# eloimoliner/audio-inpainting-diffusion

Hardware: AMD Instinct MI355X
Metric: denoiser-steps/sec (higher is better)
Workload: dtype f32; 1 GPU; BASELINE.json configs[1]: batch 8 x 22.05 kHz MAESTRO-shape segments (L=184184) per GPU, 300 ms gap, T=36 EDM schedule, Heun steps 5..16; branch=xi=0.25 (reconstruction guidance: forward + input-VJP), segments_per_gpu=8, network=unet_cqt_oct_with_attention 7-octave, 186.3 M params, random-init (seeded), sub_batch_streams=2, cu_partition=0, hip_graph_replay=False, backend=single process, visible_gpus=1

## Files before the change

audio_inpainting_diffusion_amd/_lib.py:

```python
from __future__ import annotations

import ctypes as C
import os
from typing import Optional, Sequence

import torch

_HERE = os.path.dirname(os.path.abspath(__file__))
LIB_PATH = os.path.join(_HERE, "libaid_hip.so")
if os.environ.get("AID_EXPERIMENT") == "1" and os.environ.get("AID_LIB_PATH"):
    LIB_PATH = os.environ["AID_LIB_PATH"]
    import sys as _sys
    print(f"[aid] AID_EXPERIMENT=1: loading {LIB_PATH} instead of the in-tree libaid_hip.so", file=_sys.stderr)
AID_CQT_MAX_OCT = 12
AID_STATS_SPLIT = 32
AID_CONV2D_SPLIT_FLAG_BYTES = 4096
AID_ATTN_MAX_T = 128


class AidError(RuntimeError):
    pass


class View(C.Structure):
# ... 21 lines not shown
                ("dot_ws", C.c_void_p), ("dot_n", C.c_int), ("stat_ws", C.c_void_p), ("stat_n", C.c_int),
                ("x2", View), ("Cin1", C.c_int),
                ("fin_mode", C.c_int), ("fin_count", C.c_void_p), ("fin_gamma", C.c_void_p), ("fin_mod", C.c_void_p), ("fin_mod_ld", C.c_int64),
                ("fin_eps", C.c_float), ("fin_scale", C.c_void_p), ("fin_stats", C.c_void_p)]


class Wino2dGemmParams(C.Structure):
    _fields_ = [("U", C.c_void_p), ("V", C.c_void_p), ("M", C.c_void_p), ("nxi", C.c_int), ("Cin", C.c_int), ("Cout", C.c_int),
                ("Cin_pad", C.c_int), ("Cout_pad", C.c_int), ("N", C.c_int64), ("variant", C.c_int)]


class ResampleParams(C.Structure):
    _fields_ = [("x", View), ("y", View), ("B", C.c_int), ("C", C.c_int), ("F", C.c_int), ("T", C.c_int),
                ("up", C.c_int), ("adjoint", C.c_int), ("accumulate", C.c_int)]


class AttentionParams(C.Structure):
    _fields_ = [("qk", C.c_void_p), ("v", C.c_void_p), ("out", C.c_void_p), ("probs", C.c_void_p),
                ("B", C.c_int), ("H", C.c_int), ("F", C.c_int), ("T", C.c_int), ("scale", C.c_float), ("bias", C.c_void_p)]


class EmbedParams(C.Structure):
    _fields_ = [("sigma", C.c_void_p), ("rff_freq", C.c_void_p), ("w0", C.c_void_p), ("b0", C.c_void_p),
                ("w1", C.c_void_p), ("b1", C.c_void_p), ("w2", C.c_void_p), ("b2", C.c_void_p), ("emb", C.c_void_p),
                ("B", C.c_int), ("rff", C.c_int), ("h0", C.c_int), ("h1", C.c_int), ("E", C.c_int)]


class ModulationParams(C.Structure):
    _fields_ = [("emb", C.c_void_p), ("W", C.c_void_p), ("bias", C.c_void_p), ("mod", C.c_void_p),
                ("B", C.c_int), ("E", C.c_int), ("N", C.c_int)]


class CqtTables(C.Structure):
    _fields_ = [("n_oct", C.c_int), ("bins", C.c_int), ("rc", C.c_void_p), ("Lg", C.c_void_p), ("goff", C.c_void_p),
                ("g", C.c_void_p), ("T_oct", C.c_void_p), ("twiddle", C.c_void_p), ("Tmax", C.c_int)]


class CqtParams(C.Structure):
    _fields_ = [("tab", CqtTables), ("T_host", C.c_int * AID_CQT_MAX_OCT), ("oct", View * AID_CQT_MAX_OCT),
                ("spec", C.c_void_p), ("band_ws", C.c_void_p), ("in_scale", C.c_void_p), ("B", C.c_int), ("Lh", C.c_int),
                ("unnormalized", C.c_int)]


class CqtGatherParams(C.Structure):
    _fields_ = [("band_ws", C.c_void_p), ("kfirst", C.c_void_p), ("kcount", C.c_void_p),
                ("rc", C.c_void_p), ("Lg", C.c_void_p), ("goff", C.c_void_p), ("woff", C.c_void_p), ("Tk", C.c_void_p),
                ("gdM", C.c_void_p), ("X", C.c_void_p), ("cskip", C.c_void_p), ("cout", C.c_void_p), ("hpf", C.c_void_p),
                ("Y", C.c_void_p), ("B", C.c_int), ("Lh", C.c_int), ("ws_per_b", C.c_int64), ("band_scale", C.c_void_p)]


class AxpbyParams(C.Structure):
    _fields_ = [("x", C.c_void_p), ("y", C.c_void_p), ("out", C.c_void_p), ("a", C.c_void_p), ("b", C.c_void_p),
                ("B", C.c_int), ("L", C.c_int64), ("a_host", C.c_float), ("b_host", C.c_float)]

    def __init__(self, x, y, out, a, b, B, L, a_host=1.0, b_host=1.0):
        super().__init__(x, y, out, a, b, B, L, a_host, b_host)


class ScoreStepParams(C.Structure):
    _fields_ = [("x", C.c_void_p), ("xhat", C.c_void_p), ("yobs", C.c_void_p), ("smask", C.c_void_p),
                ("smask_sB", C.c_int64), ("x0", C.c_void_p), ("d0", C.c_void_p), ("t", C.c_void_p), ("h", C.c_void_p),
                ("xnext", C.c_void_p), ("dout", C.c_void_p), ("xh_out", C.c_void_p),
                ("B", C.c_int), ("L", C.c_int64), ("mode", C.c_int), ("t_host", C.c_float), ("h_host", C.c_float)]


class Add2Params(C.Structure):
    _fields_ = [("u", View), ("v", View), ("y", View), ("B", C.c_int), ("C", C.c_int), ("F", C.c_int), ("T", C.c_int),
                ("a", C.c_float), ("b", C.c_float)]


class ScaleActParams(C.Structure):
    _fields_ = [("x", View), ("y", View), ("scale", C.c_void_p), ("scale_ld", C.c_int64),
                ("B", C.c_int), ("C", C.c_int), ("F", C.c_int), ("T", C.c_int), ("act", C.c_int), ("wino", C.c_int), ("dilF", C.c_int), ("mul", C.c_float)]


class FftPassParams(C.Structure):
    _fields_ = [("inp", C.c_void_p), ("out", C.c_void_p), ("twiddle", C.c_void_p), ("B", C.c_int), ("N", C.c_int), ("R", C.c_int),
                ("Ns", C.c_int), ("in_mode", C.c_int), ("out_mode", C.c_int), ("sign", C.c_float), ("out_scale", C.c_float)]


class GroupDotParams(C.Structure):
    _fields_ = [("u", View), ("v", View), ("B", C.c_int), ("C", C.c_int), ("F", C.c_int), ("T", C.c_int), ("groups", C.c_int),
                ("ws", C.c_void_p)]


class NormBwdParams(C.Structure):
    _fields_ = [("gd", View), ("x", View), ("gy", View), ("out", View),
                ("B", C.c_int), ("C", C.c_int), ("F", C.c_int), ("T", C.c_int), ("groups", C.c_int),
                ("stats", C.c_void_p), ("ws", C.c_void_p), ("eps", C.c_float), ("a", C.c_float), ("accumulate", C.c_int),
                ("ws_n", C.c_int), ("wout", View), ("wscale", C.c_void_p), ("wscale_ld", C.c_int64), ("wform", C.c_int), ("coef_ready", C.c_int), ("wdil", C.c_int)]


class AttentionBwdParams(C.Structure):
    _fields_ = [("qk", C.c_void_p), ("v", C.c_void_p), ("probs", C.c_void_p), ("gout", C.c_void_p),
                ("gqk", C.c_void_p), ("gv", C.c_void_p), ("B", C.c_int), ("H", C.c_int), ("F", C.c_int), ("T", C.c_int),
                ("scale", C.c_float), ("accumulate_gv", C.c_int), ("ws", C.c_void_p)]


class GuidanceSeedParams(C.Structure):
    _fields_ = [("xhat", C.c_void_p), ("y", C.c_void_p), ("mask", C.c_void_p), ("mask_sB", C.c_int64),
                ("g", C.c_void_p), ("norm", C.c_void_p), ("B", C.c_int), ("L", C.c_int64), ("norm_type", C.c_int), ("beta", C.c_float)]

    def __init__(self, xhat, y, mask, mask_sB, g, norm, B, L, norm_type=2, beta=1.0):
        super().__init__(xhat, y, mask, mask_sB, g, norm, B, L, norm_type, beta)


class GuidanceStepParams(C.Structure):
    _fields_ = [("xhat", C.c_void_p), ("g", C.c_void_p), ("out", C.c_void_p), ("step_out", C.c_void_p), ("s_out", C.c_void_p),
                ("B", C.c_int), ("L", C.c_int64), ("coef", C.c_float), ("inv_sqrt_len", C.c_float), ("eps", C.c_float)]


class SetRowsParams(C.Structure):
    _fields_ = [("out", C.c_void_p), ("ld", C.c_int64), ("B", C.c_int), ("n", C.c_int), ("v", C.c_float * 8)]


class RowNormParams(C.Structure):
    _fields_ = [("x", C.c_void_p), ("out", C.c_void_p), ("B", C.c_int), ("L", C.c_int64)]


class ResamplePolyParams(C.Structure):
    _fields_ = [("x", C.c_void_p), ("y", C.c_void_p), ("kernel", C.c_void_p), ("x_ld", C.c_int64), ("y_ld", C.c_int64),
                ("L", C.c_int64), ("Lout", C.c_int64), ("B", C.c_int), ("orig_freq", C.c_int), ("new_freq", C.c_int),
                ("width", C.c_int), ("K", C.c_int)]


class StftParams(C.Structure):
    _fields_ = [("x", C.c_void_p), ("frames", C.c_void_p), ("out", C.c_void_p),
                ("window", C.c_void_p), ("twiddle", C.c_void_p), ("inv_env", C.c_void_p),
                ("mask", C.c_void_p), ("mask_sB", C.c_int64), ("mask_ld", C.c_int64),
                ("add1", C.c_void_p), ("add2", C.c_void_p), ("c0", C.c_float),
                ("B", C.c_int), ("L", C.c_int64), ("Lp", C.c_int64),
                ("n_fft", C.c_int), ("hop", C.c_int), ("n_frames", C.c_int), ("adjoint", C.c_int)]


class WgradParams(C.Structure):
    _fields_ = [("gy", View), ("x", View), ("P", C.c_void_p),
                ("B", C.c_int), ("Cin", C.c_int), ("Cout", C.c_int), ("F", C.c_int), ("T", C.c_int), ("KH", C.c_int), ("KW", C.c_int),
                ("dilF", C.c_int), ("S", C.c_int), ("alpha", C.c_float), ("wino", C.c_int)]


class WinoGyParams(C.Structure):
    _fields_ = [("gy", View), ("out", View), ("B", C.c_int), ("C", C.c_int), ("F", C.c_int), ("T", C.c_int)]


class PackConvWeightParams(C.Structure):
    _fields_ = [("w", C.c_void_p), ("wp", C.c_void_p), ("wpT", C.c_void_p), ("wpw", C.c_void_p), ("wpwT", C.c_void_p),
                ("Cout", C.c_int), ("Cin", C.c_int), ("KH", C.c_int), ("KW", C.c_int),
                ("Cin_pad", C.c_int), ("Cout_pad", C.c_int), ("Cin_padT", C.c_int), ("Cout_padT", C.c_int),
                ("wpw8", C.c_void_p), ("wpw8T", C.c_void_p), ("wpw2", C.c_void_p), ("wpw2T", C.c_void_p), ("wpw3", C.c_void_p), ("wpw3T", C.c_void_p)]


class WgradReduceParams(C.Structure):
    _fields_ = [("P", C.c_void_p), ("W", C.c_void_p), ("gate", C.c_void_p), ("gate_ld", C.c_int64),
                ("in_scale", C.c_void_p), ("in_scale_ld", C.c_int64), ("dW", C.c_void_p), ("dgate", C.c_void_p), ("dgate_ld", C.c_int64),
                ("B", C.c_int), ("S", C.c_int), ("Cout", C.c_int), ("Cin", C.c_int), ("K", C.c_int), ("accumulate", C.c_int),
                ("wino", C.c_int), ("Uw", C.c_void_p), ("Cin_pad", C.c_int), ("Cout_pad", C.c_int)]


class ChannelDotParams(C.Structure):
    _fields_ = [("u", View), ("v", View), ("out", C.c_void_p), ("out_ld", C.c_int64),
                ("B", C.c_int), ("C", C.c_int), ("F", C.c_int), ("T", C.c_int)]


class RelposBwdParams(C.Structure):
    _fields_ = [("dS", C.c_void_p), ("bucket", C.c_void_p), ("dW", C.c_void_p),
                ("B", C.c_int), ("H", C.c_int), ("T", C.c_int), ("num_buckets", C.c_int), ("accumulate", C.c_int)]


class ScaleBwdParams(C.Structure):
    _fields_ = [("S", C.c_void_p), ("S_ld", C.c_int64), ("scale", C.c_void_p), ("scale_ld", C.c_int64), ("gamma", C.c_void_p),
                ("mod", C.c_void_p), ("mod_ld", C.c_int64), ("stats", C.c_void_p), ("dgamma", C.c_void_p), ("dmod", C.c_void_p),
                ("dmod_ld", C.c_int64), ("B", C.c_int), ("C", C.c_int), ("groups", C.c_int), ("accumulate", C.c_int)]


class ModulationBwdParams(C.Structure):
    _fields_ = [("dmod", C.c_void_p), ("emb", C.c_void_p), ("W", C.c_void_p), ("dW", C.c_void_p), ("dbias", C.c_void_p),
                ("demb", C.c_void_p), ("B", C.c_int), ("E", C.c_int), ("N", C.c_int), ("accumulate", C.c_int),
                ("part", C.c_void_p), ("part_floats", C.c_int64)]


class EmbedBwdParams(C.Structure):
    _fields_ = [("fwd", EmbedParams), ("demb", C.c_void_p), ("dw0", C.c_void_p), ("db0", C.c_void_p), ("dw1", C.c_void_p),
                ("db1", C.c_void_p), ("dw2", C.c_void_p), ("db2", C.c_void_p), ("accumulate", C.c_int)]


class AdamParams(C.Structure):
    _fields_ = [("param", C.c_void_p), ("grad", C.c_void_p), ("m", C.c_void_p), ("v", C.c_void_p), ("gscale", C.c_void_p),
                ("n", C.c_int64), ("lr", C.c_float), ("beta1", C.c_float), ("beta2", C.c_float), ("eps", C.c_float),
                ("bias1", C.c_float), ("bias2_sqrt", C.c_float)]


class EmaParams(C.Structure):
    _fields_ = [("dst", C.c_void_p), ("src", C.c_void_p), ("n", C.c_int64), ("rate", C.c_float)]


class SumsqParams(C.Structure):
    _fields_ = [("x", C.c_void_p), ("ws", C.c_void_p), ("out", C.c_void_p), ("n", C.c_int64), ("max_norm", C.c_float)]


AID_SUMSQ_BLOCKS = 512


class FirParams(C.Structure):
    _fields_ = [("x", C.c_void_p), ("out", C.c_void_p), ("h", C.c_void_p), ("add1", C.c_void_p), ("add2", C.c_void_p), ("c0", C.c_float),
                ("B", C.c_int), ("K", C.c_int), ("stride", C.c_int), ("pad_left", C.c_int), ("adjoint", C.c_int),
                ("L", C.c_int64), ("L_out", C.c_int64), ("x_ld", C.c_int64), ("out_ld", C.c_int64)]


class IirParams(C.Structure):
    _fields_ = [("x", C.c_void_p), ("out", C.c_void_p), ("pre", C.c_void_p), ("coef", C.c_void_p), ("H", C.c_void_p),
                ("z", C.c_void_p), ("state", C.c_void_p), ("add1", C.c_void_p), ("add2", C.c_void_p), ("c0", C.c_float),
                ("B", C.c_int), ("N", C.c_int), ("C", C.c_int), ("clamp", C.c_int), ("adjoint", C.c_int),
                ("L", C.c_int64), ("x_ld", C.c_int64), ("out_ld", C.c_int64)]


class ClipParams(C.Structure):
    _fields_ = [("x", C.c_void_p), ("xref", C.c_void_p), ("out", C.c_void_p), ("add1", C.c_void_p), ("add2", C.c_void_p),
                ("c0", C.c_float), ("clip", C.c_float), ("B", C.c_int), ("adjoint", C.c_int),
                ("L", C.c_int64), ("x_ld", C.c_int64), ("out_ld", C.c_int64)]


AID_DEGRADE_ABI_VERSION = 1
DEGRADE_EXPORTS = ["aid_degrade_abi_version", "aid_fir", "aid_iir", "aid_clip"]


class StftMagParams(C.Structure):
    _fields_ = [("x", C.c_void_p), ("g", C.c_void_p), ("out", C.c_void_p), ("frames", C.c_void_p), ("window", C.c_void_p), ("twiddle", C.c_void_p),
                ("B", C.c_int), ("n_fft", C.c_int), ("hop", C.c_int), ("n_frames", C.c_int), ("adjoint", C.c_int),
                ("L", C.c_int64), ("x_ld", C.c_int64), ("out_ld", C.c_int64)]


class MatrixNormParams(C.Structure):
    _fields_ = [("den", C.c_void_p), ("y", C.c_void_p), ("g", C.c_void_p), ("norm", C.c_void_p), ("r", C.c_void_p), ("diag", C.c_void_p),
                ("B", C.c_int), ("F", C.c_int), ("T", C.c_int), ("ord", C.c_int), ("max_iter", C.c_int), ("tol", C.c_double)]


AID_PHASE_ABI_VERSION = 1
PHASE_EXPORTS = ["aid_phase_abi_version", "aid_stft_mag", "aid_matrix_norm_seed"]

class ArCarryParams(C.Structure):
    _fields_ = [("x", C.c_void_p), ("y", C.c_void_p), ("out", C.c_void_p), ("B", C.c_int), ("first", C.c_int),
                ("L", C.c_int64), ("end", C.c_int64), ("off", C.c_int64), ("out_ld", C.c_int64)]


AID_AR_ABI_VERSION = 1
AR_EXPORTS = ["aid_ar_abi_version", "aid_ar_carry"]


class WindowGatherParams(C.Structure):
    _fields_ = [("rec", C.c_void_p), ("out", C.c_void_p), ("mask", C.c_void_p), ("y", C.c_void_p), ("m", C.c_void_p), ("jobs", C.c_void_p),
                ("J", C.c_int), ("R", C.c_int), ("L", C.c_int64), ("N", C.c_int64), ("rec_ld", C.c_int64), ("out_ld", C.c_int64), ("mask_ld", C.c_int64)]


class WindowScatterParams(C.Structure):
    _fields_ = [("x", C.c_void_p), ("out", C.c_void_p), ("jobs", C.c_void_p), ("J", C.c_int), ("R", C.c_int),
                ("L", C.c_int64), ("N", C.c_int64), ("out_ld", C.c_int64)]


AID_RESTORE_ABI_VERSION = 1
AID_RESTORE_JOB_FIELDS = 6
RESTORE_EXPORTS = ["aid_restore_abi_version", "aid_window_gather", "aid_window_scatter"]

class ClipKnownParams(C.Structure):
    _fields_ = [("x", C.c_void_p), ("xref", C.c_void_p), ("y", C.c_void_p), ("state", C.c_void_p), ("clip", C.c_void_p), ("out", C.c_void_p),
                ("B", C.c_int), ("mode", C.c_int), ("L", C.c_int64), ("x_ld", C.c_int64), ("xref_ld", C.c_int64), ("y_ld", C.c_int64),
                ("state_ld", C.c_int64), ("out_ld", C.c_int64)]


class DeclipGatherParams(C.Structure):
    _fields_ = [("rec", C.c_void_p), ("out", C.c_void_p), ("clip", C.c_void_p), ("y", C.c_void_p), ("k", C.c_void_p), ("c", C.c_void_p), ("jobs", C.c_void_p),
                ("J", C.c_int), ("R", C.c_int), ("L", C.c_int64), ("N", C.c_int64), ("rec_ld", C.c_int64), ("out_ld", C.c_int64)]


AID_DECLIP_ABI_VERSION = 1
DECLIP_EXPORTS = ["aid_declip_abi_version", "aid_clip_known", "aid_declip_gather"]

class ResamplePolyAdjParams(C.Structure):
    _fields_ = [("g", C.c_void_p), ("gx", C.c_void_p), ("kT", C.c_void_p), ("j_lo", C.c_void_p), ("j_hi", C.c_void_p),
                ("g_ld", C.c_int64), ("gx_ld", C.c_int64), ("L", C.c_int64), ("Lout", C.c_int64),
                ("B", C.c_int), ("orig_freq", C.c_int), ("new_freq", C.c_int), ("width", C.c_int), ("K", C.c_int)]


AID_RESAMPLE_OP_ABI_VERSION = 1
RESAMPLE_OP_EXPORTS = ["aid_resample_op_abi_version", "aid_resample_poly_adj"]

class FirObservedParams(C.Structure):
    _fields_ = [("x", C.c_void_p), ("y", C.c_void_p), ("state", C.c_void_p), ("h", C.c_void_p), ("out", C.c_void_p),
                ("B", C.c_int), ("K", C.c_int), ("mode", C.c_int), ("L", C.c_int64), ("x_ld", C.c_int64), ("y_ld", C.c_int64),
                ("state_ld", C.c_int64), ("out_ld", C.c_int64)]


class BweGatherParams(C.Structure):
    _fields_ = [("rec", C.c_void_p), ("out", C.c_void_p), ("y", C.c_void_p), ("state", C.c_void_p), ("jobs", C.c_void_p),
                ("J", C.c_int), ("R", C.c_int), ("K", C.c_int), ("L", C.c_int64), ("N", C.c_int64), ("rec_ld", C.c_int64), ("out_ld", C.c_int64)]


AID_BWE_LONG_ABI_VERSION = 1
BWE_LONG_EXPORTS = ["aid_bwe_long_abi_version", "aid_fir_observed", "aid_bwe_gather"]

EXPORTS = ["aid_abi_version", "aid_last_error", "aid_last_kernel", "aid_group_stats", "aid_conv2d", "aid_conv2d_pack_dims", "aid_conv2d_stat_partials", "aid_pack_conv_weight", "aid_wino_gy", "aid_conv2d_wgrad_tiles", "aid_resample",
           "aid_time_attention", "aid_embed", "aid_modulation", "aid_cqt_analysis", "aid_cqt_synthesis",
           "aid_cqt_gather", "aid_axpby", "aid_score_step", "aid_add2", "aid_group_dot", "aid_norm_bwd",
           "aid_time_attention_bwd", "aid_guidance_seed", "aid_guidance_step", "aid_set_rows", "aid_row_norm", "aid_scale_act", "aid_fft_pass",
           "aid_stft_frames", "aid_stft_ola", "aid_resample_poly", "aid_conv2d_wino_input_supported", "aid_conv2d_dot_partials", "aid_conv2d_x2_supported", "aid_conv2d_dot_partials_1x1", "aid_conv2d_wino_input_ok", "aid_conv2d_wino_form", "aid_conv2d_wino8_supported", "aid_conv2d_wino_split_ws_bytes", "aid_conv2d_fin_supported",
           "aid_conv2d_wgrad", "aid_wgrad_reduce", "aid_channel_dot", "aid_relpos_bwd", "aid_scale_bwd", "aid_modulation_bwd", "aid_embed_bwd",
           "aid_adam", "aid_ema", "aid_sumsq", "aid_wino2d_gemm", "aid_wino2d_set_split", "aid_conv2d_wino2d_gemm", "aid_conv2d_wino2d_output", "aid_conv2d_wino2d_supported", "aid_conv2d_wino2d_positions", "aid_conv2d_wino2d_wanted", "aid_conv2d_wino2d_tform"]

_lib = None


def lib():
    global _lib
    if _lib is None:
        if not os.path.exists(LIB_PATH):
            raise AidError(f"{LIB_PATH} not found: build the HIP extension first (python __graft_entry__.py). "
                           "There is no CPU / eager fallback on the product path.")
        L = C.CDLL(LIB_PATH)
        L.aid_last_error.restype = C.c_char_p
        L.aid_abi_version.restype = C.c_int
        L.aid_last_kernel.restype = C.c_char_p
        for name in EXPORTS:
            if not hasattr(L, name):
                raise AidError(f"libaid_hip.so does not export {name}")
        L.aid_conv2d_pack_dims.argtypes = [C.c_int, C.c_int, C.POINTER(C.c_int), C.POINTER(C.c_int)]
        L.aid_conv2d_pack_dims.restype = None
        L.aid_conv2d_wino_input_supported.argtypes = [C.c_int, C.c_int, C.c_int]
        L.aid_conv2d_wino_input_supported.restype = C.c_int
        L.aid_conv2d_dot_partials.argtypes = [C.c_int] * 7
        L.aid_conv2d_dot_partials.restype = C.c_int
        L.aid_conv2d_x2_supported.argtypes = [C.c_int] * 5
        L.aid_conv2d_x2_supported.restype = C.c_int
        L.aid_conv2d_dot_partials_1x1.argtypes = [C.c_int] * 5
        L.aid_conv2d_dot_partials_1x1.restype = C.c_int
        L.aid_conv2d_wino_input_ok.argtypes = [C.c_int] * 6
        L.aid_conv2d_wino_input_ok.restype = C.c_int
        L.aid_conv2d_wino8_supported.argtypes = [C.c_int] * 5
        L.aid_conv2d_wino8_supported.restype = C.c_int
        L.aid_conv2d_fin_supported.argtypes = [C.c_int] * 7
        L.aid_conv2d_fin_supported.restype = C.c_int
        L.aid_conv2d_wino_form.argtypes = [C.c_int] * 6
        L.aid_conv2d_wino_form.restype = C.c_int
        L.aid_conv2d_wino_split_ws_bytes.argtypes = [C.c_int] * 6
        L.aid_conv2d_wino_split_ws_bytes.restype = C.c_int64
        L.aid_conv2d_stat_partials.argtypes = [C.c_int] * 7
        L.aid_conv2d_stat_partials.restype = C.c_int
        L.aid_conv2d_wgrad_tiles.argtypes = [C.c_int] * 5
        L.aid_conv2d_wgrad_tiles.restype = C.c_int
        L.aid_conv2d_wino2d_supported.argtypes = [C.c_int] * 5
        L.aid_conv2d_wino2d_supported.restype = C.c_int
        L.aid_conv2d_wino2d_wanted.argtypes = [C.c_int] * 6
        L.aid_conv2d_wino2d_wanted.restype = C.c_int
        L.aid_conv2d_wino2d_tform.argtypes = [C.c_int] * 6
        L.aid_conv2d_wino2d_tform.restype = C.c_int
        L.aid_conv2d_wino2d_positions.argtypes = [C.c_int] * 4
        L.aid_conv2d_wino2d_positions.restype = C.c_int64
        L.aid_wino2d_set_split.argtypes = [C.c_int]
        L.aid_wino2d_set_split.restype = C.c_int
        for name in EXPORTS[3:]:
            if name not in ("aid_conv2d_pack_dims", "aid_conv2d_wino_input_supported", "aid_conv2d_dot_partials", "aid_conv2d_x2_supported", "aid_conv2d_dot_partials_1x1", "aid_conv2d_wino_input_ok", "aid_conv2d_wino_form", "aid_conv2d_wino8_supported", "aid_conv2d_wino_split_ws_bytes", "aid_conv2d_fin_supported",
                            "aid_conv2d_stat_partials", "aid_conv2d_wgrad_tiles", "aid_conv2d_wino2d_supported", "aid_conv2d_wino2d_positions", "aid_conv2d_wino2d_wanted", "aid_conv2d_wino2d_tform", "aid_wino2d_set_split"):
                getattr(L, name).argtypes = [C.c_void_p, C.c_void_p]
                getattr(L, name).restype = C.c_int
        if L.aid_abi_version() != 14:
            raise AidError("ABI version mismatch")
        for name in DEGRADE_EXPORTS:
            if not hasattr(L, name):
                raise AidError(f"libaid_hip.so does not export {name}")
            getattr(L, name).argtypes = [C.c_void_p, C.c_void_p]
            getattr(L, name).restype = C.c_int
        L.aid_degrade_abi_version.argtypes = []
        if L.aid_degrade_abi_version() != AID_DEGRADE_ABI_VERSION:
            raise AidError("include/aid_degrade.h ABI version mismatch")
        for name in PHASE_EXPORTS:
            if not hasattr(L, name):
                raise AidError(f"libaid_hip.so does not export {name}")
            getattr(L, name).argtypes = [C.c_void_p, C.c_void_p]
            getattr(L, name).restype = C.c_int
        L.aid_phase_abi_version.argtypes = []
        if L.aid_phase_abi_version() != AID_PHASE_ABI_VERSION:
            raise AidError("include/aid_phase.h ABI version mismatch")
        for name in AR_EXPORTS:
            if not hasattr(L, name):
                raise AidError(f"libaid_hip.so does not export {name}")
            getattr(L, name).argtypes = [C.c_void_p, C.c_void_p]
            getattr(L, name).restype = C.c_int
        L.aid_ar_abi_version.argtypes = []
        if L.aid_ar_abi_version() != AID_AR_ABI_VERSION:
            raise AidError("include/aid_autoregressive.h ABI version mismatch")
        for name in RESTORE_EXPORTS:
            if not hasattr(L, name):
                raise AidError(f"libaid_hip.so does not export {name}")
            getattr(L, name).argtypes = [C.c_void_p, C.c_void_p]
            getattr(L, name).restype = C.c_int
        L.aid_restore_abi_version.argtypes = []
        if L.aid_restore_abi_version() != AID_RESTORE_ABI_VERSION:
            raise AidError("include/aid_restore.h ABI version mismatch")
        for name in DECLIP_EXPORTS:
            if not hasattr(L, name):
                raise AidError(f"libaid_hip.so does not export {name}")
            getattr(L, name).argtypes = [C.c_void_p, C.c_void_p]
            getattr(L, name).restype = C.c_int
        L.aid_declip_abi_version.argtypes = []
        if L.aid_declip_abi_version() != AID_DECLIP_ABI_VERSION:
            raise AidError("include/aid_declip.h ABI version mismatch")
        for name in RESAMPLE_OP_EXPORTS:
            if not hasattr(L, name):
                raise AidError(f"libaid_hip.so does not export {name}")
            getattr(L, name).argtypes = [C.c_void_p, C.c_void_p]
            getattr(L, name).restype = C.c_int
        L.aid_resample_op_abi_version.argtypes = []
        if L.aid_resample_op_abi_version() != AID_RESAMPLE_OP_ABI_VERSION:
            raise AidError("include/aid_resample_op.h ABI version mismatch")
        for name in BWE_LONG_EXPORTS:
            if not hasattr(L, name):
                raise AidError(f"libaid_hip.so does not export {name}")
            getattr(L, name).argtypes = [C.c_void_p, C.c_void_p]
            getattr(L, name).restype = C.c_int
        L.aid_bwe_long_abi_version.argtypes = []
        if L.aid_bwe_long_abi_version() != AID_BWE_LONG_ABI_VERSION:
            raise AidError("include/aid_bwe_long.h ABI version mismatch")
        _lib = L
    return _lib


def _stream() -> int:
    return torch.cuda.current_stream().cuda_stream


def call(name: str, params) -> None:
    rc = getattr(lib(), name)(C.addressof(params), _stream())
    if rc != 0:
        raise AidError(f"{name} failed rc={rc}: {lib().aid_last_error().decode()}")


def call_on(fn, params_addr: int, stream: int, name: str = "") -> None:
    rc = fn(params_addr, stream)
    if rc != 0:
        raise AidError(f"{name} failed rc={rc}: {lib().aid_last_error().decode()}")


def _req(t: torch.Tensor):
    if not (t.is_cuda and t.dtype == torch.float32):
        raise AidError("HIP kernels need float32 tensors on the GPU (no CPU fallback)")


def ptr(t: Optional[torch.Tensor]) -> Optional[int]:
    return None if t is None else t.data_ptr()


def view4(t: Optional[torch.Tensor]) -> View:
    if t is None:
        return View(None, 0, 0, 0)
    _req(t)
    assert t.dim() == 4 and (t.stride(3) == 1 or t.shape[3] == 1), "T must be contiguous"
    return View(t.data_ptr(), t.stride(0), t.stride(1), t.stride(2))


def pack_dims(cin: int, cout: int):
    a, b = C.c_int(0), C.c_int(0)
    lib().aid_conv2d_pack_dims(cin, cout, C.byref(a), C.byref(b))
    return a.value, b.value


def pack_conv_weight(w: torch.Tensor, transpose: bool = False) -> torch.Tensor:
    if w.dim() == 2:
        w = w[:, :, None, None]
    elif w.dim() == 3:
        w = w[:, :, None, :]
    w = w.detach().float()
    if transpose:
        w = w.flip(2, 3).permute(1, 0, 2, 3)
    co, ci, kh, kw = w.shape
    cip, cop = pack_dims(ci, co)
    out = torch.zeros(kh * kw, cip, cop, device=w.device, dtype=torch.float32)
    out[:, :ci, :co] = w.permute(2, 3, 1, 0).reshape(kh * kw, ci, co)
    return out


def pack_conv_weight_wino(w: torch.Tensor, transpose: bool = False) -> torch.Tensor:
    w = w.detach().double()
    if transpose:
        w = w.flip(2, 3).permute(1, 0, 2, 3)
    co, ci, kh, kw = w.shape
    assert (kh, kw) == (5, 3)
    w0, w1, w2 = w[..., 0], w[..., 1], w[..., 2]
    U = torch.stack((w0 / 4, -(w0 + w1 + w2) / 6, -(w0 - w1 + w2) / 6, (w0 + 2 * w1 + 4 * w2) / 24,
                     (w0 - 2 * w1 + 4 * w2) / 24, w2), dim=0)
    nxi = U.shape[0]
    cip, cop = pack_dims(ci, co)
    out = torch.zeros(nxi * kh, cip, cop, device=w.device, dtype=torch.float32)
    out[:, :ci, :co] = U.permute(0, 3, 2, 1).reshape(nxi * kh, ci, co).float()
    return out


W8_POINTS = (0.4, 0.8, 1.25, 2.5)


def wino8_matrices():
    import numpy as np
    n = 10
    pts = np.array([0.0] + [sg * a for a in W8_POINTS for sg in (1, -1)], dtype=np.float64)

    def vander(cols):
        V = np.zeros((n, cols))
        for j in range(n - 1):
            V[j] = pts[j] ** np.arange(cols)
        V[n - 1, cols - 1] = 1.0
        return V
    AT, G, BT = vander(8).T, vander(3), np.linalg.inv(vander(n)).T
    sc = np.abs(BT).max(axis=1)
    BT = BT / sc[:, None]
    BT[np.abs(BT) < 1e-13] = 0.0
    return AT, G * sc[:, None], BT


def wino45_matrices():
    import numpy as np

    def toom(points, m, r):
        n = m + r - 1
        pts = np.array([0.0] + [sg * a for a in points for sg in (1, -1)], dtype=np.float64)

        def vander(cols):
            V = np.zeros((n, cols))
            for j in range(n - 1):
                V[j] = pts[j] ** np.arange(cols)
            V[n - 1, cols - 1] = 1.0
            return V
        AT, G, BT = vander(m).T, vander(r), np.linalg.inv(vander(n)).T
        sc = np.abs(BT).max(axis=1)
        BT = BT / sc[:, None]
        BT[np.abs(BT) < 1e-13] = 0.0
        return AT, G * sc[:, None], BT
    return toom((1.0, 2.0, 0.5), 4, 5) + toom((1.0, 2.0), 4, 3)


def pack_conv_weight_wino2d(w: torch.Tensor, transpose: bool = False) -> torch.Tensor:
    w = w.detach().double()
    if transpose:
        w = w.flip(2, 3).permute(1, 0, 2, 3)
    co, ci, kh, kw = w.shape
    assert (kh, kw) == (5, 3)
    m = wino45_matrices()
    GF, GT = torch.from_numpy(m[1]).to(w.device), torch.from_numpy(m[4]).to(w.device)
    U = torch.einsum("fh,tk,oihk->ftio", GF, GT, w).reshape(48, ci, co)
    cip, cop = pack_dims(ci, co)
    out = torch.zeros(48, cip, cop, device=w.device, dtype=torch.float32)
    out[:, :ci, :co] = U.float()
    return out


def pack_conv_weight_wino2d8(w: torch.Tensor, transpose: bool = False) -> torch.Tensor:
    w = w.detach().double()
    if transpose:
        w = w.flip(2, 3).permute(1, 0, 2, 3)
    co, ci, kh, kw = w.shape
    assert (kh, kw) == (5, 3)
    GF = torch.from_numpy(wino45_matrices()[1]).to(w.device)
    G8 = torch.from_numpy(wino8_matrices()[1]).to(w.device)
    U = torch.einsum("fh,tk,oihk->ftio", GF, G8, w).reshape(80, ci, co)
    cip, cop = pack_dims(ci, co)
    out = torch.zeros(80, cip, cop, device=w.device, dtype=torch.float32)
    out[:, :ci, :co] = U.float()
    return out


def pack_conv_weight_wino8(w: torch.Tensor, transpose: bool = False) -> torch.Tensor:
    w = w.detach().double()
    if transpose:
        w = w.flip(2, 3).permute(1, 0, 2, 3)
    co, ci, kh, kw = w.shape
    assert (kh, kw) == (5, 3)
    G = torch.from_numpy(wino8_matrices()[1]).to(w.device)
    U = torch.einsum("xk,oihk->xoih", G, w)
    cip, cop = pack_dims(ci, co)
    out = torch.zeros(10 * kh, cip, cop, device=w.device, dtype=torch.float32)
    out[:, :ci, :co] = U.permute(0, 3, 2, 1).reshape(10 * kh, ci, co).float()
    return out


def _cqt_params(tr, tab, octs: Sequence[torch.Tensor], window: Optional[torch.Tensor] = None) -> CqtParams:
    P = tr.plan
    p = CqtParams()
    p.tab = CqtTables(P.numocts, P.binsoct, ptr(tab["rc"]), ptr(tab["Lg"]), ptr(tab["goff"]),
                      ptr(tab["g"] if window is None else window), ptr(tab["T_oct"]), ptr(tab["twiddle"]), P.Tmax)
    for o in range(P.numocts):
        p.T_host[o] = int(P.T_oct[o])
        t = octs[o]
        _req(t)
        assert t.shape[1] == 2 and t.shape[2] == P.binsoct and t.shape[3] == P.T_oct[o] and t.stride(3) == 1
        p.oct[o] = View(t.data_ptr(), t.stride(0), t.stride(1), t.stride(2))
    p.B = octs[0].shape[0]
    p.Lh = P.Lh
    p.unnormalized = 0
    return p


def cqt_analysis(tr, tab, spec_ri: torch.Tensor, octs, in_scale=None, window=None, unnormalized=False):
    _req(spec_ri)
    assert spec_ri.is_contiguous()
    p = _cqt_params(tr, tab, octs, window)
    p.spec = spec_ri.data_ptr()
    p.in_scale = ptr(in_scale)
    p.unnormalized = int(unnormalized)
    call("aid_cqt_analysis", p)


def cqt_synthesis(tr, tab, octs, ws: torch.Tensor):
    p = _cqt_params(tr, tab, octs)
    p.band_ws = ws.data_ptr()
    call("aid_cqt_synthesis", p)


def cqt_gather(tr, tab, ws, Y, X=None, cskip=None, cout=None, hpf=None, window=None, band_scale=None):
    P = tr.plan
    p = CqtGatherParams(ptr(ws), ptr(tab["kfirst"]), ptr(tab["kcount"]), ptr(tab["rc"]), ptr(tab["Lg"]),
                        ptr(tab["goff"]), ptr(tab["woff"]), ptr(tab["Tk"]), ptr(tab["gdM"] if window is None else window),
                        ptr(X), ptr(cskip), ptr(cout), ptr(hpf), Y.data_ptr(), Y.shape[0], P.Lh, P.ws_per_b, ptr(band_scale))
    call("aid_cqt_gather", p)
```

audio_inpainting_diffusion_amd/csrc/aid_conv.hip:

```cpp
#include "aid_common.h"
#include "aid_mfma_dma.h"
#include "aid_conv1x1_plan.h"
#include <stdlib.h>

struct ConvDev {
    aid_conv2d_params p;
    int tt_log2;
    int rows_log2;
    int tiles_t;
    int nrows;
    int nchunks;
    int splits, cps;
    float* ws;
};

__device__ __forceinline__ float4 xform4(float4 v, float sc, int act) {
    v.x *= sc; v.y *= sc; v.z *= sc; v.w *= sc;
    if (act == 1) { v.x = aid_gelu(v.x); v.y = aid_gelu(v.y); v.z = aid_gelu(v.z); v.w = aid_gelu(v.w); }
    return v;
}

template <int KH, int KW, int MT, int NT, int WGM, int WGN, int KC>
__global__ __launch_bounds__(64 * WGM * WGN) void conv_mfma_kernel(const ConvDev a) {
    constexpr int NTHREADS = 64 * WGM * WGN;
// ... 137 lines not shown
            const bool ok = xg[i] >= 0 && c < p.Cin;
            xv[i] = ok ? *reinterpret_cast<const float4*>(p.x.p + xg[i] + (int64_t)c * p.x.sC) : make_float4(0.f, 0.f, 0.f, 0.f);
            xs[i] = (ok && p.in_scale) ? p.in_scale[xsc[i] + c] : 1.f;
        }
        if (KW > 1) {
#pragma unroll
            for (int i = 0; i < HQ; ++i) {
                const int c = c0 + hci[i];
                const bool ok = hg[i] >= 0 && c < p.Cin;
                float v = ok ? p.x.p[hg[i] + (int64_t)c * p.x.sC] : 0.f;
                if (ok && p.in_scale) v *= p.in_scale[hsc[i] + c];
                hv[i] = v;
            }
        }
#pragma unroll
        for (int i = 0; i < WQ; ++i)
            wv[i] = (wg[i] >= 0) ? *reinterpret_cast<const float4*>(wbase + wg[i] + (int64_t)c0 * p.Cout_pad)
                                 : make_float4(0.f, 0.f, 0.f, 0.f);
    };
    auto write_slot = [&](float* Xs, float* Ws, int slot) {
#pragma unroll
        for (int i = 0; i < XQ; ++i)
            if ((slot < 0 || (i % (NSLOT - 1)) == slot) && (XQ_TOTAL % NTHREADS == 0 || xlds[i] >= 0))
                *reinterpret_cast<float4*>(Xs + xlds[i]) = xform4(xv[i], xs[i], p.act);
#pragma unroll
        for (int i = 0; i < WQ; ++i)
            if ((slot < 0 || (i % (NSLOT - 1)) == slot) && wlds[i] >= 0)
                *reinterpret_cast<float4*>(Ws + wlds[i]) = wv[i];
        if (KW > 1 && (slot < 0 || slot == NSLOT - 2)) {
#pragma unroll
            for (int i = 0; i < HQ; ++i)
                if (hlds[i] >= 0) Xs[hlds[i]] = (p.act == 1) ? aid_gelu(hv[i]) : hv[i];
        }
    };
    auto halo_slow = [&](float* Xs, int c0) {
        for (int h = tid; h < 2 * nstrips; h += NTHREADS) {
            const int s = h >> 1, side = h & 1;
            const int kh = s % KH;
            const int s2 = s / KH;
            const int rr = s2 & (ROWS - 1);
            const int ci = s2 >> a.rows_log2;
            const int b = rowinfo[2 * rr];
            const int fi = rowinfo[2 * rr + 1] + (kh - KH / 2) * p.dilF;
            const int t = side ? (t0 + TT) : (t0 - 1);
            const int c = c0 + ci;
            float v = 0.f;
            if (b >= 0 && fi >= 0 && fi < p.F && c < p.Cin && t >= 0 && t < p.T) {
                v = p.x.p[(int64_t)b * p.x.sB + (int64_t)c * p.x.sC + (int64_t)fi * p.x.sF + t];
                if (p.in_scale) v *= p.in_scale[(int64_t)b * p.in_scale_ld + c];
                if (p.act == 1) v = aid_gelu(v);
            }
            Xs[s * TTP + (side ? 4 + TT : 3)] = v;
        }
    };

    const int cb = (int)blockIdx.z * a.cps;
    const int nloc = (a.nchunks - cb < a.cps) ? (a.nchunks - cb) : a.cps;
    issue_loads(cb * KC);
    write_slot(smem, smem + XSZ, -1);
    if (KW > 1 && !halo_fast) halo_slow(smem, cb * KC);
    __syncthreads();

    for (int ch = 0; ch < nloc; ++ch) {
        const int cur = ch & 1;
        const float* Xs = smem + cur * BUFSZ;
        const float* Ws = Xs + XSZ;
        float* Xn = smem + (cur ^ 1) * BUFSZ;
        float* Wn = Xn + XSZ;
        const bool more = (ch + 1) < nloc;
        float av[2][MT], bv[2][NT];
        auto load_frags = [&](int ks, int buf) {
            const int tap = ks / (KC / 2);
            const int cp = ks % (KC / 2);
            const int kh = tap / KW, kw = tap % KW;
            const int ci = 2 * cp + ci_lane;
#pragma unroll
            for (int i = 0; i < MT; ++i)
                av[buf][i] = Ws[(tap * KC + ci) * M_BLK + (wm * MT + i) * 32 + (lane & 31)];
#pragma unroll
            for (int j = 0; j < NT; ++j)
                bv[buf][j] = Xs[ci * strip_ci + kh * TTP + xoff[j] + kw];
        };
        load_frags(0, 0);
#pragma unroll
        for (int slot = 0; slot < NSLOT; ++slot) {
            if (slot == 0) __builtin_amdgcn_s_setprio(3);
            else if (slot == 1) __builtin_amdgcn_s_setprio(2);
            else if (slot == 2) __builtin_amdgcn_s_setprio(1);
            else __builtin_amdgcn_s_setprio(0);
#pragma unroll
            for (int k = 0; k < KS_PER_SLOT; ++k) {
                const int ks = slot * KS_PER_SLOT + k;
                if (ks + 1 < KSTEPS) load_frags(ks + 1, (ks + 1) & 1);
#pragma unroll
                for (int i = 0; i < MT; ++i)
#pragma unroll
                    for (int j = 0; j < NT; ++j)
                        acc[i][j] = __builtin_amdgcn_mfma_f32_32x32x2f32(av[ks & 1][i], bv[ks & 1][j], acc[i][j], 0, 0, 0);
                if (slot == 0 && k == 0 && more) issue_loads((cb + ch + 1) * KC);
            }
            if (more && slot > 0) write_slot(Xn, Wn, slot - 1);
        }
        if (more && KW > 1 && !halo_fast) halo_slow(Xn, (cb + ch + 1) * KC);
        __syncthreads();
    }

#pragma unroll
    for (int j = 0; j < NT; ++j) {
        const int n = (wn * NT + j) * 32 + (lane & 31);
        const int rr = n >> a.tt_log2;
        const int tt = n & (TT - 1);
        const int b = rowinfo[2 * rr];
        const int f = rowinfo[2 * rr + 1];
        const int t = t0 + tt;
        if (b < 0 || t >= p.T) continue;
        if (a.splits > 1) {
            const int64_t ft = (int64_t)p.F * p.T;
            float* wsb = a.ws + (((int64_t)blockIdx.z * p.B + b) * p.Cout) * ft + (int64_t)f * p.T + t;
#pragma unroll
            for (int i = 0; i < MT; ++i) {
                const int mbase = m0 + (wm * MT + i) * 32 + 4 * (lane >> 5);
#pragma unroll
                for (int r = 0; r < 16; ++r) {
                    const int m = mbase + (r & 3) + 8 * (r >> 2);
                    if (m < p.Cout) wsb[(int64_t)m * ft] = acc[i][j][r];
                }
            }
            continue;
        }
        const int64_t ybase = (int64_t)b * p.y.sB + (int64_t)f * p.y.sF + t;
        const int64_t rbase = p.res.p ? ((int64_t)b * p.res.sB + (int64_t)f * p.res.sF + t) : 0;
        const int64_t abase = p.aux.p ? ((int64_t)b * p.aux.sB + (int64_t)f * p.aux.sF + t) : 0;
#pragma unroll
        for (int i = 0; i < MT; ++i) {
            float rv[16], uv[16], sv[16];
            const int mbase = m0 + (wm * MT + i) * 32 + 4 * (lane >> 5);
#pragma unroll
            for (int r = 0; r < 16; ++r) {
                const int m = mbase + (r & 3) + 8 * (r >> 2);
                const bool ok = m < p.Cout;
                rv[r] = (ok && p.res.p) ? p.res.p[rbase + (int64_t)m * p.res.sC] : 0.f;
                sv[r] = (ok && p.out_scale) ? p.out_scale[(int64_t)b * p.out_scale_ld + m] : 1.f;
                uv[r] = (ok && p.epi == 1) ? p.aux.p[abase + (int64_t)m * p.aux.sC] * p.aux_scale[(int64_t)b * p.aux_scale_ld + m] : 0.f;
            }
#pragma unroll
            for (int r = 0; r < 16; ++r) {
                const int m = mbase + (r & 3) + 8 * (r >> 2);
                if (m >= p.Cout) continue;
                float v = acc[i][j][r] * sv[r];
                if (p.epi == 1) v *= aid_dgelu(uv[r]);
                v += p.res_scale * rv[r];
                p.y.p[ybase + (int64_t)m * p.y.sC] = p.alpha * v;
            }
        }
    }
}

__global__ __launch_bounds__(256) void conv_splitk_reduce_kernel(const aid_conv2d_params p, const float* __restrict__ ws, int splits) {
    const int64_t ft = (int64_t)p.F * p.T;
    const int64_t q4 = ft >> 2;
    const int64_t total = (int64_t)p.B * p.Cout * q4;
    const int64_t i = (int64_t)blockIdx.x * 256 + threadIdx.x;
    if (i >= total) return;
    const int64_t bm = i / q4, e = (i - bm * q4) * 4;
    const int b = (int)(bm / p.Cout), m = (int)(bm - (int64_t)b * p.Cout);
    const int f = (int)(e / p.T), t = (int)(e - (int64_t)f * p.T);
    const int64_t plane = (int64_t)p.B * p.Cout * ft;
    float4 s = make_float4(0.f, 0.f, 0.f, 0.f);
    for (int z = 0; z < splits; ++z) {
        const float4 v = *reinterpret_cast<const float4*>(ws + z * plane + bm * ft + e);
        s.x += v.x; s.y += v.y; s.z += v.z; s.w += v.w;
    }
    const float sc = p.out_scale ? p.out_scale[(int64_t)b * p.out_scale_ld + m] : 1.f;
    float4 r = make_float4(0.f, 0.f, 0.f, 0.f);
    if (p.res.p) r = *reinterpret_cast<const float4*>(p.res.p + (int64_t)b * p.res.sB + (int64_t)m * p.res.sC + (int64_t)f * p.res.sF + t);
    float4 o;
    o.x = p.alpha * (p.res_scale * r.x + s.x * sc); o.y = p.alpha * (p.res_scale * r.y + s.y * sc);
    o.z = p.alpha * (p.res_scale * r.z + s.z * sc); o.w = p.alpha * (p.res_scale * r.w + s.w * sc);
    *reinterpret_cast<float4*>(p.y.p + (int64_t)b * p.y.sB + (int64_t)m * p.y.sC + (int64_t)f * p.y.sF + t) = o;
}

int aid_conv_splitk_reduce(const aid_conv2d_params* p, const float* ws, int splits, hipStream_t st) {
    const int64_t total = (int64_t)p->B * p->Cout * ((int64_t)p->F * p->T / 4);
    hipLaunchKernelGGL(conv_splitk_reduce_kernel, dim3((unsigned)((total + 255) / 256)), dim3(256), 0, st, *p, ws, splits);
    AID_CHECK_LAUNCH();
    return AID_OK;
}

bool aid_conv_splitk_scratch_ok(const aid_conv2d_params* p, int S) {
    return p->ws && c11_splitk_fits(S, p->B, p->Cout, p->F, p->T, p->ws_bytes) && aid_view_aligned(p->y, 4) && (!p->res.p || aid_view_aligned(p->res, 4));
}

extern "C" void aid_conv2d_pack_dims(int Cin, int Cout, int* Cin_pad, int* Cout_pad) {
    const int mb = c11_pick_mblk(Cout);
    *Cin_pad = ((Cin + 31) / 32) * 32;
    *Cout_pad = ((Cout + mb - 1) / mb) * mb;
}

template <int KH, int KW, int MT, int NT, int WGM, int WGN, int KC>
static int launch_cfg(const aid_conv2d_params* p, hipStream_t st, int splits = 1) {
    constexpr int M_BLK = 32 * MT * WGM;
    constexpr int N_BLK = 32 * NT * WGN;
    ConvDev a;
    a.p = *p;
    int TT = aid_pow2ceil(p->T);
    if (TT > N_BLK) TT = N_BLK;
    if (TT < 4) TT = 4;
    a.tt_log2 = aid_ilog2(TT);
    const int ROWS = N_BLK / TT;
    a.rows_log2 = aid_ilog2(ROWS);
    a.tiles_t = aid_cdiv(p->T, TT);
    a.nrows = p->B * p->F;
    a.nchunks = aid_cdiv(p->Cin, KC);
    a.cps = aid_cdiv(a.nchunks, splits);
    a.splits = aid_cdiv(a.nchunks, a.cps);
    a.ws = p->ws;
    const int rgroups = aid_cdiv(a.nrows, ROWS);
    dim3 grid((unsigned)(rgroups * a.tiles_t), (unsigned)(p->Cout_pad / M_BLK), (unsigned)a.splits);
    const size_t lds = sizeof(float) * 2 * ((size_t)KC * ROWS * KH * (TT + (KW > 1 ? 8 : 0)) + (size_t)KH * KW * KC * M_BLK) +
                       sizeof(int) * 2 * ROWS;
    AID_REQUIRE(lds <= 160 * 1024, "aid_conv2d: LDS tile too large");
    auto kern = conv_mfma_kernel<KH, KW, MT, NT, WGM, WGN, KC>;
    static bool attr_set = false;
    if (!attr_set) {
        (void)hipFuncSetAttribute((const void*)kern, hipFuncAttributeMaxDynamicSharedMemorySize, 160 * 1024);
        attr_set = true;
    }
    hipLaunchKernelGGL(kern, grid, dim3(64 * WGM * WGN), lds, st, a);
    AID_CHECK_LAUNCH();
    aid_note_kernel(a.splits > 1 ? "conv_mfma_kernel+splitk" : (KH == 5 ? "conv_mfma_kernel(5x3)" : "conv_mfma_kernel(1x1)"));
    if (a.splits > 1) return aid_conv_splitk_reduce(p, (const float*)p->ws, a.splits, st);
    return AID_OK;
}

static int launch_m53(const aid_conv2d_params* p, hipStream_t st) {
    int mb = c11_pick_mblk(p->Cout);
    if (mb == 128) {
        const int64_t npos = (int64_t)p->B * p->F * p->T;
        const int64_t ntiles = (npos + 255) / 256;
        if (ntiles * (p->Cout_pad / 128) < 192) mb = (ntiles * (p->Cout_pad / 64) < 192) ? 32 : 64;
    }
    switch (mb) {
        case 32: return launch_cfg<5, 3, 1, 2, 1, 4, 4>(p, st);
        case 64:
            if (p->T >= 64) return launch_cfg<5, 3, 1, 2, 2, 8, 4>(p, st);
            return launch_cfg<5, 3, 2, 2, 1, 4, 4>(p, st);
        case 96: return launch_cfg<5, 3, 1, 2, 3, 4, 4>(p, st);
        default: return launch_cfg<5, 3, 1, 2, 4, 4, 4>(p, st);
    }
}

template <int KC>
static int launch_m11(const aid_conv2d_params* p, hipStream_t st) {
    C11Shape s = c11_shape_of(*p);
    C11Plan pl = c11_tiled_plan(s);
    if (pl.S > 1 && !aid_conv_splitk_scratch_ok(p, pl.S)) {
        s.ws = false;
        pl = c11_tiled_plan(s);
    }
    AID_REQUIRE(pl.ok, "aid_conv2d: too many rows or tiles for the tiled 1x1 kernel");
    if (pl.S > 1) return launch_cfg<1, 1, 1, 2, 2, 4, KC>(p, st, pl.S);
    switch (pl.WGM) {
        case 1: return launch_cfg<1, 1, 1, 2, 1, 4, KC>(p, st);
        case 2: return launch_cfg<1, 1, 1, 2, 2, 4, KC>(p, st);
        case 3: return launch_cfg<1, 1, 1, 2, 3, 4, KC>(p, st);
        default: return launch_cfg<1, 1, 1, 2, 4, 4, KC>(p, st);
    }
}

int aid_conv53_dma_try(const aid_conv2d_params* p, hipStream_t st);
int aid_conv53_wino_try(const aid_conv2d_params* p, hipStream_t st);
int aid_conv53_wino2d(const aid_conv2d_params* p, hipStream_t st);
int aid_conv1x1_stream_try(const aid_conv2d_params* p, hipStream_t st);
int aid_conv1x1_dma_try(const aid_conv2d_params* p, hipStream_t st);
int aid_conv_small_try(const aid_conv2d_params* p, hipStream_t st);
int aid_conv1x1_rs_try(const aid_conv2d_params* p, hipStream_t st);

static int conv1x1_dispatch(const aid_conv2d_params* p, hipStream_t st, const char* only_first_two) {
    int r = aid_conv1x1_rs_try(p, st);
    if (r == 0) r = aid_conv1x1_dma_try(p, st);
    if (r == 0 && only_first_two) {
        aid_set_error(only_first_two);
        return AID_E_BADARG;
    }
    if (r == 0) r = aid_conv1x1_stream_try(p, st);
    if (r != 0) return r < 0 ? r : AID_OK;
    return p->Cin <= 8 ? launch_m11<8>(p, st) : launch_m11<16>(p, st);
}

static C11Shape c11_query_shape(int B, int Cin, int Cout, int F, int T) {
    C11Shape s = {};
    int cip;
    aid_conv2d_pack_dims(Cin, Cout, &cip, &s.Cout_pad);
    s.B = B; s.Cin = Cin; s.Cout = Cout; s.F = F; s.T = T;
    return s;
}

extern "C" int aid_conv2d_dot_partials_1x1(int B, int Cin, int Cout, int F, int T) {
    C11Shape s = c11_query_shape(B, Cin, Cout, F, T);
    s.epi = 1; s.dot = true;
    return c11_plan(s).slots;
}

extern "C" int aid_conv2d_x2_supported(int Cin, int Cin1, int Cout, int F, int T) {
    C11Shape s = c11_query_shape(1, Cin, Cout, F, T);
    s.x2 = true; s.Cin1 = Cin1;
    return c11_dma_plan(s).family ? 1 : 0;
}

extern "C" int aid_conv2d(const aid_conv2d_params* p, void* stream) {
    hipStream_t st = (hipStream_t)stream;
    AID_REQUIRE(p && p->x.p && p->y.p && p->wp, "aid_conv2d: null pointer");
    AID_REQUIRE(p->B > 0 && p->Cin > 0 && p->Cout > 0 && p->F > 0 && p->T > 0, "aid_conv2d: empty shape");
    AID_REQUIRE((p->T % 4) == 0, "aid_conv2d: T must be a multiple of 4");
    AID_REQUIRE(p->x_wino == 3 || p->x_wino == 4 || aid_view_strides(p->x, 4), "aid_conv2d: input view strides % 4 == 0");
    AID_REQUIRE((((uintptr_t)p->x.p) & 15) == 0, "aid_conv2d: input view must be 16-byte aligned");
    int cip, cop;
    aid_conv2d_pack_dims(p->Cin, p->Cout, &cip, &cop);
    AID_REQUIRE(p->Cin_pad == cip && p->Cout_pad == cop, "aid_conv2d: packed weight dims mismatch (use aid_conv2d_pack_dims)");
    AID_REQUIRE(p->epi == 0 || (p->epi == 1 && p->aux.p && p->aux_scale), "aid_conv2d: epi=1 needs aux + aux_scale");
    AID_REQUIRE((int64_t)p->B * p->in_scale_ld < (1LL << 31), "aid_conv2d: in_scale too large");
    AID_REQUIRE(!p->x_wino || (p->KH == 5 && p->KW == 3 && p->wp_wino), "aid_conv2d: x_wino is a 5x3 Winograd-path input layout");
    AID_REQUIRE(!p->fin_mode || (p->x_wino && p->KH == 5 && p->KW == 3), "aid_conv2d: fin_mode is an option of the row-shared 5x3 Winograd kernels (aid_conv2d_fin_supported)");
    if (p->x_wino == 3 || p->x_wino == 4) return aid_conv53_wino2d(p, st);
    if (p->x2.p) {
        AID_REQUIRE(p->KH == 1 && p->KW == 1 && !p->in_scale && p->act == 0 && p->Cin1 > 0 && p->Cin1 < p->Cin && (p->Cin1 % 16) == 0 && ((p->Cin - p->Cin1) % 16) == 0,
                    "aid_conv2d: x2 is an option of plain 1x1 convolutions with both K segments multiples of 16");
        return conv1x1_dispatch(p, st, "aid_conv2d: x2 given but the layer is not eligible for the 1x1 kernels that take it");
    }
    if (p->stat_ws) {
        AID_REQUIRE(!p->dot_ws && p->epi == 0 && p->x_wino, "aid_conv2d: stat_ws is an option of the forward epilogue on Winograd-domain input");
        AID_REQUIRE(p->stat_n > 0 && p->stat_n == aid_conv2d_stat_partials(p->B, p->Cin, p->Cout, p->F, p->T, p->dilF, p->x_wino), "aid_conv2d: stat_n != aid_conv2d_stat_partials()");
    }
    if (p->dot_ws && p->KH == 1 && p->KW == 1) {
        AID_REQUIRE(p->epi == 1 && !p->res.p, "aid_conv2d: dot_ws on a 1x1 layer is an option of the dGELU epilogue without residual");
        return conv1x1_dispatch(p, st, "aid_conv2d: dot_ws given but the 1x1 layer is not eligible (aid_conv2d_dot_partials_1x1)");
    }
    if (p->dot_ws) {
        AID_REQUIRE(p->KH == 5 && p->KW == 3 && p->wp_wino && p->wino_taps == (p->x_wino == 2 ? 50 : 30) && p->epi == 1 && !p->res.p,
                    "aid_conv2d: dot_ws is an option of the F(4,3) / F(8,3) dGELU epilogue");
        AID_REQUIRE(p->dot_n > 0 && p->dot_n == aid_conv2d_dot_partials(p->B, p->Cin, p->Cout, p->F, p->T, p->dilF, p->x_wino), "aid_conv2d: dot_n != aid_conv2d_dot_partials()");
        const int r = aid_conv53_wino_try(p, st);
        if (r == 0) aid_set_error("aid_conv2d: dot_ws given but the layer is not eligible for the F(4,3) kernels");
        return r == 1 ? AID_OK : (r < 0 ? r : AID_E_BADARG);
    }
    if (p->x_wino) {
        const int r = aid_conv53_wino_try(p, st);
        return r == 1 ? AID_OK : (r < 0 ? r : AID_E_BADARG);
    }
    if (p->Cin <= 8 || p->Cout <= 8) {
        const int r = aid_conv_small_try(p, st);
        if (r != 0) return r < 0 ? r : AID_OK;
    }
    if (p->KH == 5 && p->KW == 3) {
        if (p->wp_wino) {
            const int r = aid_conv53_wino_try(p, st);
            if (r != 0) return r < 0 ? r : AID_OK;
        }
        {
            const int r = aid_conv53_dma_try(p, st);
            if (r != 0) return r < 0 ? r : AID_OK;
        }
        return launch_m53(p, st);
    }
    if (p->KH == 1 && p->KW == 1) return conv1x1_dispatch(p, st, nullptr);
    aid_set_error("aid_conv2d: unsupported kernel size (5x3 and 1x1 only)");
    return AID_E_BADARG;
}
```

audio_inpainting_diffusion_amd/csrc/aid_conv1x1_dma.hip:

```cpp
#include "aid_common.h"
#include "aid_mfma_dma.h"
#include "aid_conv1x1_plan.h"
#include <type_traits>

int aid_conv_splitk_reduce(const aid_conv2d_params* p, const float* ws, int splits, hipStream_t st);
bool aid_conv_splitk_scratch_ok(const aid_conv2d_params* p, int S);

struct C11Dev {
    aid_conv2d_params p;
    const float* zero;
    int tt_log2, rows_log2, tiles_t, nrows, nchunks;
    int nx, ny, per_xcd;
    int nch1;
    int splits, cps;
    float* ws;
};

__device__ float4 g_aid_zero_page_c11[16];

template <int MT, int WGM, int WGN, int RMAX, int KC, int MINW>
__global__ __launch_bounds__(64 * WGM * WGN, MINW) void conv11_dma_kernel(const C11Dev a) {
    constexpr int NT = 2;
    constexpr int NW = WGM * WGN;
    constexpr int NTHREADS = 64 * NW;
    constexpr int M_BLK = 32 * MT * WGM;
    constexpr int N_BLK = 32 * NT * WGN;
    constexpr int XSZ = KC * N_BLK;
    constexpr int WROW = (M_BLK % 64 == 0) ? M_BLK : ((M_BLK + 63) / 64) * 64;
    constexpr int WSZ = KC * WROW;
    constexpr int BUFSZ = XSZ + WSZ;
    constexpr int NXP = XSZ / 256;
    constexpr int NWP = WSZ / 256;
    constexpr int NP = NXP + NWP;
    constexpr int PPW = (NP + NW - 1) / NW;
    constexpr int NSTEP = KC / 2;
    static_assert(N_BLK % 256 == 0 && WSZ % 256 == 0, "whole 1-KiB pieces");

    const aid_conv2d_params& p = a.p;
    const int TT = 1 << a.tt_log2;
    const int ROWS = 1 << a.rows_log2;

    __shared__ __attribute__((aligned(16))) float sbuf0[BUFSZ];
    __shared__ __attribute__((aligned(16))) float sbuf1[BUFSZ];
    __shared__ int rowinfo[2 * RMAX];

    const int tid = threadIdx.x;
    const int lane = tid & 63;
    const int wave = __builtin_amdgcn_readfirstlane(tid >> 6);
    const int wm = wave / WGN;
    const int wn = wave % WGN;

    const int Lt = (blockIdx.x & 7) * a.per_xcd + (blockIdx.x >> 3);
    if (Lt >= a.nx * a.ny) return;
    const int bx = Lt / a.ny;
    const int by = Lt - bx * a.ny;
    const int tile_t = bx % a.tiles_t;
    const int rg = bx / a.tiles_t;
    const int row0 = rg << a.rows_log2;
    const int t0 = tile_t << a.tt_log2;
    const int m0 = by * M_BLK;

    for (int r = tid; r < ROWS; r += NTHREADS) {
        const int rid = row0 + r;
        int b = -1, f = 0;
        if (rid < a.nrows) { b = rid / p.F; f = rid - b * p.F; }
        rowinfo[2 * r] = b;
        rowinfo[2 * r + 1] = f;
    }
    __syncthreads();

    const float* psrc[PPW];
    const float* psrc2[PPW];
    int pstride[PPW], pstride2[PPW], plds[PPW];
#pragma unroll
    for (int i = 0; i < PPW; ++i) {
        const int pc = wave + i * NW;
        psrc[i] = a.zero; pstride[i] = 0; plds[i] = -1;
        psrc2[i] = a.zero; pstride2[i] = 0;
        if (pc < NXP) {
            const int ci = pc / (N_BLK / 256), sub = pc % (N_BLK / 256);
            const int n = sub * 256 + 4 * lane;
            const int rr = n >> a.tt_log2, tt = n & (TT - 1);
            const int b = rowinfo[2 * rr];
            const int f = rowinfo[2 * rr + 1];
            plds[i] = ci * N_BLK + sub * 256;
            if (b >= 0 && t0 + tt < p.T) {
                psrc[i] = p.x.p + (int64_t)b * p.x.sB + (int64_t)ci * p.x.sC + (int64_t)f * p.x.sF + t0 + tt;
                pstride[i] = (int)(KC * p.x.sC);
                if (p.x2.p) {
                    psrc2[i] = p.x2.p + (int64_t)b * p.x2.sB + (int64_t)ci * p.x2.sC + (int64_t)f * p.x2.sF + t0 + tt;
                    pstride2[i] = (int)(KC * p.x2.sC);
                }
            }
        } else if (pc < NP) {
            const int wp_ = pc - NXP;
            const int e = wp_ * 256 + 4 * lane;
            const int ci = e / WROW, col = e % WROW;
            plds[i] = XSZ + wp_ * 256;
            if (col < M_BLK) {
                psrc[i] = p.wp + (int64_t)ci * p.Cout_pad + m0 + col;
                pstride[i] = KC * p.Cout_pad;
                psrc2[i] = psrc[i] + (int64_t)a.nch1 * pstride[i];
                pstride2[i] = pstride[i];
            }
        }
    }
    const int half = lane >> 5;
    const int vB = half * N_BLK + wn * 64 + 2 * (lane & 31);
    int vA[MT];
#pragma unroll
    for (int i = 0; i < MT; ++i) vA[i] = XSZ + half * WROW + (wm * MT + i) * 32 + (lane & 31);
    const int b_tile = rowinfo[0];
    const float* sp = (p.in_scale && b_tile >= 0) ? p.in_scale + (int64_t)b_tile * p.in_scale_ld + half : nullptr;

    f32x16 acc[MT][NT];
#pragma unroll
    for (int i = 0; i < MT; ++i)
#pragma unroll
        for (int j = 0; j < NT; ++j)
#pragma unroll
            for (int r = 0; r < 16; ++r) acc[i][j][r] = 0.f;

    auto issue_dma = [&](int ch, float* buf) {
#pragma unroll
        for (int i = 0; i < PPW; ++i) {
            if (plds[i] >= 0) {
                const float* src = ch < a.nch1 ? psrc[i] + (int64_t)ch * pstride[i] : psrc2[i] + (int64_t)(ch - a.nch1) * pstride2[i];
                AID_GLDS16(src, buf + plds[i]);
            }
        }
    };
    float sc[2][NSTEP];
    auto load_scales = [&](int ch, int q) {
#pragma unroll
        for (int s = 0; s < NSTEP; ++s) {
            const int ci = ch * KC + 2 * s + half;
            sc[q][s] = (sp && ci < p.Cin) ? sp[ch * KC + 2 * s] : 1.f;
        }
    };

    const int ch_lo = blockIdx.y * a.cps;
    const int ch_hi = min(a.nchunks, ch_lo + a.cps);
    issue_dma(ch_lo, sbuf0);
    load_scales(ch_lo, 0);
    __syncthreads();

    auto chunk = [&](auto curc, int ch) {
        constexpr int cur = decltype(curc)::value;
        const float* Bf = cur ? sbuf1 : sbuf0;
        float* Nx = cur ? sbuf0 : sbuf1;
        const bool more = (ch + 1) < ch_hi;
        if (more) { issue_dma(ch + 1, Nx); load_scales(ch + 1, cur ^ 1); }
        float2 bv[2];
        float av[2][MT];
        auto load_step = [&](int s, int buf) {
            bv[buf] = *reinterpret_cast<const float2*>(Bf + vB + 2 * s * N_BLK);
#pragma unroll
            for (int i = 0; i < MT; ++i) av[buf][i] = Bf[vA[i] + 2 * s * WROW];
        };
        load_step(0, 0);
#pragma unroll
        for (int s = 0; s < NSTEP; ++s) {
            if (s + 1 < NSTEP) load_step(s + 1, (s + 1) & 1);
            const int bq = s & 1;
#pragma unroll
            for (int i = 0; i < MT; ++i) {
                const float aw = av[bq][i] * sc[cur][s];
                acc[i][0] = __builtin_amdgcn_mfma_f32_32x32x2f32(aw, bv[bq].x, acc[i][0], 0, 0, 0);
                acc[i][1] = __builtin_amdgcn_mfma_f32_32x32x2f32(aw, bv[bq].y, acc[i][1], 0, 0, 0);
            }
        }
        __syncthreads();
    };
    for (int ch = ch_lo; ch < ch_hi; ch += 2) {
        chunk(std::integral_constant<int, 0>{}, ch);
        if (ch + 1 < ch_hi) chunk(std::integral_constant<int, 1>{}, ch + 1);
    }

    const int n = wn * 64 + 2 * (lane & 31);
    const int rr = n >> a.tt_log2, tt = n & (TT - 1);
    const int b = rowinfo[2 * rr];
    const int f = rowinfo[2 * rr + 1];
    const int t = t0 + tt;
    const bool live = !(b < 0 || t >= p.T);
    if (!live && !p.dot_ws) return;
    if (live && a.splits > 1) {
        const int64_t ft = (int64_t)p.F * p.T;
        float* wsb = a.ws + (((int64_t)blockIdx.y * p.B + b) * p.Cout) * ft + (int64_t)f * p.T + t;
#pragma unroll
        for (int i = 0; i < MT; ++i) {
            const int mbase = m0 + (wm * MT + i) * 32 + 4 * half;
#pragma unroll
            for (int r = 0; r < 16; ++r) {
                const int m = mbase + (r & 3) + 8 * (r >> 2);
                if (m < p.Cout) *reinterpret_cast<float2*>(wsb + (int64_t)m * ft) = make_float2(acc[i][0][r], acc[i][1][r]);
            }
        }
    }
    if (a.splits > 1) return;
    const int64_t ybase = (int64_t)b * p.y.sB + (int64_t)f * p.y.sF + t;
    const int64_t rbase = p.res.p ? ((int64_t)b * p.res.sB + (int64_t)f * p.res.sF + t) : 0;
    const int64_t abase = p.aux.p ? ((int64_t)b * p.aux.sB + (int64_t)f * p.aux.sF + t) : 0;
    float dsum[MT][4];
#pragma unroll
    for (int i = 0; i < MT; ++i)
#pragma unroll
        for (int q = 0; q < 4; ++q) dsum[i][q] = 0.f;
#pragma unroll
    for (int i = 0; i < MT; ++i) {
        if (!live) break;
        const int mbase = m0 + (wm * MT + i) * 32 + 4 * half;
#pragma unroll
        for (int r0 = 0; r0 < 16; r0 += 4) {
            float2 rv[4], uv[4];
            float sv[4], as[4];
#pragma unroll
            for (int q = 0; q < 4; ++q) {
                const int r = r0 + q;
                const int m = mbase + (r & 3) + 8 * (r >> 2);
                const bool ok = m < p.Cout;
                rv[q] = (ok && p.res.p) ? *reinterpret_cast<const float2*>(p.res.p + rbase + (int64_t)m * p.res.sC) : make_float2(0.f, 0.f);
                sv[q] = (ok && p.out_scale) ? p.out_scale[(int64_t)b * p.out_scale_ld + m] : 1.f;
                if (ok && p.epi == 1) {
                    as[q] = p.aux_scale[(int64_t)b * p.aux_scale_ld + m];
                    uv[q] = *reinterpret_cast<const float2*>(p.aux.p + abase + (int64_t)m * p.aux.sC);
                } else { as[q] = 0.f; uv[q] = make_float2(0.f, 0.f); }
            }
#pragma unroll
            for (int q = 0; q < 4; ++q) {
                const int r = r0 + q;
                const int m = mbase + (r & 3) + 8 * (r >> 2);
                if (m >= p.Cout) continue;
                float y0 = acc[i][0][r] * sv[q], y1 = acc[i][1][r] * sv[q];
                if (p.epi == 1) { y0 *= aid_dgelu(uv[q].x * as[q]); y1 *= aid_dgelu(uv[q].y * as[q]); }
                y0 += p.res_scale * rv[q].x;
                y1 += p.res_scale * rv[q].y;
                y0 *= p.alpha; y1 *= p.alpha;
                *reinterpret_cast<float2*>(p.y.p + ybase + (int64_t)m * p.y.sC) = make_float2(y0, y1);
                if (p.dot_ws) dsum[i][r0 >> 2] += y0 * uv[q].x + y1 * uv[q].y;
            }
        }
    }
    if (p.dot_ws) {
#pragma unroll
        for (int i = 0; i < MT; ++i)
#pragma unroll
            for (int q = 0; q < 4; ++q) {
                float v = live ? dsum[i][q] : 0.f;
#pragma unroll
                for (int off = 16; off >= 1; off >>= 1) v += __shfl_xor(v, off, 32);
                dsum[i][q] = v;
            }
        float* red = sbuf0;
        if ((lane & 31) == 0) {
#pragma unroll
            for (int i = 0; i < MT; ++i)
#pragma unroll
                for (int q = 0; q < 4; ++q) red[((wave * 2 + half) * MT + i) * 4 + q] = dsum[i][q];
        }
        __syncthreads();
        const int cpg = p.Cout >> 3;
        const int grp = m0 / cpg + tid;
        if (tid < M_BLK / cpg && grp < 8) {
            float sacc = 0.f;
            for (int w = 0; w < NW; ++w)
                for (int h = 0; h < 2; ++h)
                    for (int i = 0; i < MT; ++i)
                        for (int q = 0; q < 4; ++q) {
                            const int mrow = m0 + ((w / WGN) * MT + i) * 32 + 4 * h + 8 * q;
                            if (mrow < p.Cout && mrow / cpg == grp) sacc += red[((w * 2 + h) * MT + i) * 4 + q];
                        }
            const int bt = rowinfo[0];
            const int ptile = ((row0 - bt * p.F) >> a.rows_log2) * a.tiles_t + tile_t;
            p.dot_ws[((int64_t)bt * 8 + grp) * p.dot_n + ptile] = (double)sacc;
        }
    }
}

template <int MT, int WGM, int WGN, int RMAX, int KC, int MINW>
static int launch_c11(const aid_conv2d_params* p, hipStream_t st, const C11Plan& pl) {
    static const float* zero = nullptr;
    if (!zero) {
        void* z = nullptr;
        if (hipGetSymbolAddress(&z, HIP_SYMBOL(g_aid_zero_page_c11)) != hipSuccess) { aid_set_error("aid_conv2d: zero page lookup failed"); return AID_E_LAUNCH; }
        zero = (const float*)z;
    }
    C11Dev a;
    a.p = *p;
    a.zero = zero;
    a.tt_log2 = aid_ilog2(pl.TT);
    a.rows_log2 = aid_ilog2(pl.ROWS);
    a.tiles_t = pl.tiles_t;
    a.nrows = pl.nrows;
    a.nchunks = pl.nchunks;
    a.nch1 = pl.nch1;
    a.nx = pl.nx;
    a.ny = pl.ny;
    a.per_xcd = (int)(((int64_t)a.nx * a.ny + 7) / 8);
    a.cps = pl.kps / KC;
    a.splits = aid_cdiv(a.nchunks, a.cps);
    a.ws = (float*)p->ws;
    hipLaunchKernelGGL((conv11_dma_kernel<MT, WGM, WGN, RMAX, KC, MINW>), dim3((unsigned)(8 * a.per_xcd), (unsigned)a.splits), dim3(64 * WGM * WGN), 0, st, a);
    AID_CHECK_LAUNCH();
    aid_note_kernel(a.splits > 1 ? "conv11_dma_kernel+splitk" : "conv11_dma_kernel");
    if (a.splits > 1) return aid_conv_splitk_reduce(p, (const float*)p->ws, a.splits, st);
    return AID_OK;
}

template <int NT>
__global__ __launch_bounds__(256) void gemm_skinny_kernel(const aid_conv2d_params p, float* __restrict__ ws, int kps) {
    constexpr int U = 8;
    const int lane = threadIdx.x & 63, wave = threadIdx.x >> 6;
    const int m0 = (blockIdx.x * 4 + wave) * 32;
    if (m0 >= p.Cout_pad) return;
    const int half = lane >> 5, l31 = lane & 31;
    const int k0 = blockIdx.y * kps, k1 = min(p.Cin, k0 + kps);
    const float* wp = p.wp + m0 + l31;
    const float* xq[NT];
    bool ok[NT];
#pragma unroll
    for (int j = 0; j < NT; ++j) {
        const int n = j * 32 + l31;
        const int b = n / p.T, t = n - b * p.T;
        ok[j] = b < p.B;
        xq[j] = p.x.p + (ok[j] ? ((int64_t)b * p.x.sB + t) : 0);
    }
    f32x16 acc[NT];
#pragma unroll
    for (int j = 0; j < NT; ++j)
#pragma unroll
        for (int r = 0; r < 16; ++r) acc[j][r] = 0.f;
    for (int kk = k0; kk < k1; kk += 2 * U) {
        float a[U], bv[U][NT];
#pragma unroll
        for (int u = 0; u < U; ++u) {
            const int k = kk + 2 * u + half;
            const bool kin = k < k1;
            a[u] = kin ? wp[(int64_t)k * p.Cout_pad] : 0.f;
#pragma unroll
            for (int j = 0; j < NT; ++j) bv[u][j] = (kin && ok[j]) ? xq[j][(int64_t)k * p.x.sC] : 0.f;
        }
#pragma unroll
        for (int u = 0; u < U; ++u)
#pragma unroll
            for (int j = 0; j < NT; ++j) acc[j] = __builtin_amdgcn_mfma_f32_32x32x2f32(a[u], bv[u][j], acc[j], 0, 0, 0);
    }
    const int64_t ft = p.T;
#pragma unroll
    for (int j = 0; j < NT; ++j) {
        const int n = j * 32 + l31;
        const int b = n / p.T, t = n - b * p.T;
        if (b >= p.B) continue;
        float* wsb = ws + (((int64_t)blockIdx.y * p.B + b) * p.Cout) * ft + t;
#pragma unroll
        for (int r = 0; r < 16; ++r) {
            const int m = m0 + 4 * half + (r & 3) + 8 * (r >> 2);
            if (m < p.Cout) wsb[(int64_t)m * ft] = acc[j][r];
        }
    }
}

int aid_conv1x1_dma_try(const aid_conv2d_params* p, hipStream_t st) {
    if (!(p->KH == 1 && p->KW == 1)) return 0;
    C11Shape s = c11_shape_of(*p);
    C11Plan pl = c11_dma_plan(s);
    if (!pl.family) return 0;
    if (!aid_view_aligned(p->x, 4) || !aid_view_aligned(p->y, 2) || (p->res.p && !aid_view_aligned(p->res, 2)) || (p->aux.p && !aid_view_aligned(p->aux, 2))) return 0;
    if ((int64_t)4 * 16 * p->x.sC >= (1LL << 31)) return 0;
    if (p->x2.p && (!aid_view_aligned(p->x2, 4) || (int64_t)4 * 16 * p->x2.sC >= (1LL << 31))) return 0;
    if (p->dot_ws && p->dot_n != pl.slots) return 0;
    if (pl.S > 1 && !aid_conv_splitk_scratch_ok(p, pl.S)) {
        s.ws = false;
        pl = c11_dma_plan(s);
    }
    int rc;
    if (pl.family == C11_SKINNY) {
        const dim3 grid((unsigned)pl.gx, (unsigned)pl.S);
        switch (pl.nt) {
            case 1: hipLaunchKernelGGL(gemm_skinny_kernel<1>, grid, dim3(256), 0, st, *p, (float*)p->ws, pl.kps); break;
            case 2: hipLaunchKernelGGL(gemm_skinny_kernel<2>, grid, dim3(256), 0, st, *p, (float*)p->ws, pl.kps); break;
            case 3: hipLaunchKernelGGL(gemm_skinny_kernel<3>, grid, dim3(256), 0, st, *p, (float*)p->ws, pl.kps); break;
            default: hipLaunchKernelGGL(gemm_skinny_kernel<4>, grid, dim3(256), 0, st, *p, (float*)p->ws, pl.kps); break;
        }
        AID_CHECK_LAUNCH();
        aid_note_kernel("gemm_skinny_kernel+splitk");
        rc = aid_conv_splitk_reduce(p, (const float*)p->ws, pl.S, st);
    } else if (pl.MT == 2) rc = launch_c11<2, 2, 4, 16, 16, 4>(p, st, pl);
    else if (pl.MT == 1) rc = launch_c11<1, 2, 4, 16, 16, 4>(p, st, pl);
    else                 rc = launch_c11<3, 1, 4, 16, 16, 2>(p, st, pl);
    return rc == AID_OK ? 1 : rc;
}
```

audio_inpainting_diffusion_amd/csrc/aid_conv1x1_plan.h:

```cpp
#pragma once
#include <stdint.h>
#include <stdlib.h>

enum { C11_TILED = 0, C11_RS, C11_DMA, C11_SKINNY, C11_DMA_SPLITK, C11_STREAM };

struct C11Shape {
    int B, Cin, Cin1, Cout, Cout_pad, F, T;
    int act, epi;
    bool in_scale, res, x2, dot;
    bool ws;
    int64_t ws_bytes;
};

struct C11Plan {
    int family;
    bool ok;
    int MT, KMAX, key, WGM, KC;
    int slots;
    int TT, ROWS, tiles_t, nrows, nx, ny, nchunks, nch1;
    int S, kps;
    int tps, ntiles, gx;
    int nsteps1;
    int nt, mchunks;
    int64_t npos, pblocks;
};

static inline int64_t c11_cdiv(int64_t a, int64_t b) { return (a + b - 1) / b; }

static inline int c11_pick_mblk(int Cout) {
    if (Cout <= 32) return 32;
    if (Cout <= 64) return 64;
    if (Cout <= 96 || (Cout % 96 == 0 && Cout % 128 != 0)) return 96;
    return 128;
}

static inline bool c11_splitk_fits(int S, int B, int Cout, int F, int T, int64_t ws_bytes) {
    if (S < 1 || B < 1 || Cout < 1 || F < 1 || T < 1 || ws_bytes < 0) return false;
    return (int64_t)S <= ws_bytes / 4 / T / F / Cout / B;
}

static inline void c11_gemm_k_partition(int Cin, int* S, int* kps) {
    int s = 8;
    if (s > Cin / 64) s = Cin / 64;
    if (s < 1) s = 1;
    int cps = (int)c11_cdiv(c11_cdiv(Cin, 16), s);
    cps += cps & 1;
    *kps = cps * 16;
    *S = (int)c11_cdiv(Cin, *kps);
}

static inline bool c11_rs_enabled() {
#ifdef AID_EXPERIMENT
    static const int enabled = getenv("AID_C11_RS") ? atoi(getenv("AID_C11_RS")) : 1;
    return enabled != 0;
#else
    return true;
#endif
}

static inline C11Plan c11_none() { C11Plan pl = {}; pl.ok = true; return pl; }

static inline C11Plan c11_rs_plan(const C11Shape& s) {
    C11Plan pl = c11_none();
    if (!c11_rs_enabled() || s.ws || (s.act && !s.in_scale) || s.Cout != s.Cout_pad) return pl;
    if (s.F <= 1 || s.Cin < 32 || (s.Cin % 32) || s.Cin > 256 || s.Cout < 32) return pl;
    if (!(s.Cout_pad == 96 || (s.Cout_pad == 64 && s.Cin <= 64))) return pl;
    const int64_t ft = (int64_t)s.F * s.T;
    if ((s.T % 2) || (ft % 64)) return pl;
    if (ft / 64 > INT32_MAX) return pl;
    const int64_t ntiles = s.B * (ft / 64);
    if (ntiles + 8 * 256 > INT32_MAX) return pl;
    if (s.x2 && ((s.Cin1 % 2) || s.Cin1 <= 0 || s.Cin1 >= s.Cin || s.in_scale || s.act)) return pl;
    const int key = (s.act ? 8 : 0) | (s.in_scale ? 4 : 0) | (s.epi == 1 ? 2 : 0) | (s.res ? 1 : 0);
    if (!(key <= 6 || key == 12 || key == 13)) return pl;
    if (s.dot && s.epi != 1) return pl;
    const int MT = s.Cout_pad / 32;
    pl.MT = MT; pl.KMAX = (MT == 3 && s.Cin > 128) ? 256 : 128; pl.key = key;
    pl.tps = (int)(ft / 64);
    pl.ntiles = (int)ntiles;
    pl.nsteps1 = (s.x2 ? s.Cin1 : s.Cin) / 2;
    pl.ny = s.Cout_pad / (32 * MT);
    const int cap = pl.ny > 1 ? 256 / pl.ny + (256 % pl.ny ? 1 : 0) : 256;
    pl.gx = (int)c11_cdiv(ntiles, 8);
    if (pl.gx > cap) pl.gx = cap;
    pl.slots = s.dot ? pl.tps : 0;
    pl.family = C11_RS;
    return pl;
}

static inline C11Plan c11_dma_plan(const C11Shape& s) {
    C11Plan pl = c11_none();
    if (s.act != 0 || s.Cin < 32 || (s.Cin % 16) || s.Cout < 32) return pl;
    const bool gemm = s.F == 1;
    if (gemm && (s.epi != 0 || s.in_scale || s.x2 || (s.Cout_pad % 128) || s.Cin < 256)) return pl;
    if ((s.T % 4) || s.T < 8) return pl;
    if (s.x2 && ((s.Cin1 % 16) || s.Cin1 <= 0 || s.Cin1 >= s.Cin || s.in_scale)) return pl;
    int TT = 8;
    while (TT < 256 && TT < s.T) TT *= 2;
    const int ROWS = 256 / TT;
    if (ROWS > 16 || (s.in_scale && (s.F % ROWS))) return pl;
    const int mblk = (s.Cout_pad % 128 == 0) ? 128 : ((s.Cout_pad % 64 == 0) ? 64 : ((s.Cout_pad % 96 == 0) ? 96 : 0));
    if (!mblk) return pl;
    const int tiles_t = (int)c11_cdiv(s.T, TT);
    if (s.dot) {
        const int cpg = s.Cout / 8;
        if (s.epi != 1 || s.x2 || gemm || (s.Cout % 8) || (cpg % 4) || (mblk % cpg) || (s.F % ROWS)) return pl;
        if ((int64_t)(s.F / ROWS) * tiles_t > INT32_MAX) return pl;
        pl.slots = (s.F / ROWS) * tiles_t;
    }
    const int64_t nrows = (int64_t)s.B * s.F;
    const int64_t nx = nrows > INT32_MAX ? INT32_MAX : c11_cdiv(nrows, ROWS) * tiles_t;
    if (nx > (INT32_MAX - 7) / (s.Cout_pad / mblk)) { pl.slots = 0; return pl; }
    pl.TT = TT; pl.ROWS = ROWS; pl.tiles_t = tiles_t;
    pl.nrows = (int)nrows; pl.nx = (int)nx; pl.ny = s.Cout_pad / mblk;
    pl.nchunks = s.Cin / 16;
    pl.nch1 = s.x2 ? s.Cin1 / 16 : pl.nchunks;
    pl.S = 1; pl.kps = s.Cin;
    pl.MT = mblk == 128 ? 2 : (mblk == 64 ? 1 : 3);
    pl.family = C11_DMA;
    if (gemm) {
        int S, kps;
        c11_gemm_k_partition(s.Cin, &S, &kps);
        if (S > 1 && s.ws && c11_splitk_fits(S, s.B, s.Cout, s.F, s.T, s.ws_bytes)) {
            pl.S = S; pl.kps = kps;
            pl.family = C11_DMA_SPLITK;
            if ((int64_t)s.B * s.T <= 128) {
                pl.family = C11_SKINNY;
                pl.nt = (int)c11_cdiv((int64_t)s.B * s.T, 32);
                pl.gx = (int)c11_cdiv(s.Cout_pad / 32, 4);
            }
        }
    }
    return pl;
}

static inline C11Plan c11_stream_plan(const C11Shape& s) {
    C11Plan pl = c11_none();
    if (s.act != 0 || s.Cin < 16 || (s.Cin & 1) || s.Cout < 32) return pl;
    const int64_t ft = (int64_t)s.F * s.T;
    if (s.F == 1 || s.B > INT64_MAX / ft || s.B * ft < 2048) return pl;
    if (!(s.Cin <= 96 || s.Cout_pad <= 32)) return pl;
    int nt = 4;
    if ((ft % 128) || (s.T % 4)) nt = 2;
    if ((ft % (32 * nt)) || (s.T % nt)) return pl;
    const int mt32 = s.Cout_pad / 32;
    const int MT = nt == 4 ? (mt32 % 2 == 0 ? 2 : 1) : (mt32 % 4 == 0 ? 4 : (mt32 % 3 == 0 ? 3 : (mt32 % 2 == 0 ? 2 : 1)));
    pl.npos = s.B * ft;
    pl.mchunks = mt32 / MT;
    pl.pblocks = c11_cdiv(pl.npos, 4 * 32 * nt);
    if (pl.pblocks > INT32_MAX / pl.mchunks) return pl;
    pl.nt = nt;
    pl.MT = MT;
    pl.family = C11_STREAM;
    return pl;
}

static inline C11Plan c11_tiled_plan(const C11Shape& s) {
    C11Plan pl = c11_none();
    const int KC = s.Cin <= 8 ? 8 : 16;
    int mb = c11_pick_mblk(s.Cout);
    pl.S = 1;
    const int64_t nrows = (int64_t)s.B * s.F;
    int TT = 4;
    while (TT < 256 && TT < s.T) TT *= 2;
    pl.ok = nrows <= INT32_MAX && c11_cdiv(nrows, 256 / TT) * c11_cdiv(s.T, TT) <= INT32_MAX;
    if (pl.ok && mb == 128) {
        int64_t ntiles = c11_cdiv(nrows * s.T, 256);
        if (ntiles > 384) ntiles = 384;
        const int64_t wg64 = ntiles * (s.Cout_pad / 64);
        if (s.ws && s.epi == 0 && wg64 < 384 && s.Cin >= 16 * KC && s.Cout_pad % 64 == 0 && (s.T % 4) == 0) {
            int S = (int)((768 + wg64 - 1) / wg64);
            if (S > 8) S = 8;
            if (S > 1 && c11_splitk_fits(S, s.B, s.Cout, s.F, s.T, s.ws_bytes)) { pl.S = S; mb = 64; }
        }
        if (pl.S == 1 && ntiles * (s.Cout_pad / 128) < 192) mb = (ntiles * (s.Cout_pad / 64) < 192) ? 32 : 64;
    }
    pl.WGM = mb / 32; pl.KC = KC;
    return pl;
}

static inline C11Plan c11_plan(const C11Shape& s) {
    C11Plan pl = c11_rs_plan(s);
    if (!pl.family) pl = c11_dma_plan(s);
    if (!pl.family && (s.x2 || s.dot)) pl.ok = false;
    else if (!pl.family) pl = c11_stream_plan(s);
    if (!pl.family && pl.ok) pl = c11_tiled_plan(s);
    return pl;
}

template <class P> static inline C11Shape c11_shape_of(const P& p) {
    C11Shape s = {p.B, p.Cin, p.Cin1, p.Cout, p.Cout_pad, p.F, p.T, p.act, p.epi, p.in_scale != nullptr, p.res.p != nullptr, p.x2.p != nullptr, p.dot_ws != nullptr,
                  p.ws != nullptr, p.ws_bytes};
    return s;
}
```

audio_inpainting_diffusion_amd/csrc/aid_conv1x1_rs.hip:

```cpp
#include "aid_common.h"
#include "aid_mfma_dma.h"
#include "aid_conv1x1_plan.h"

struct C11RDev {
    aid_conv2d_params p;
    int nsteps;
    int nsteps1;
    int tps;
    int ntiles;
};

template <int MT, int KMAX, bool ACT, bool SCALE, bool EPI, bool RES>
__global__ __launch_bounds__(512, 1) void conv11_rs_kernel(const C11RDev a) {
    constexpr int U = 16;
    constexpr int WROW = 32 * MT;
    const aid_conv2d_params& p = a.p;
    __shared__ __attribute__((aligned(16))) float wl[KMAX * WROW];

    const int tid = threadIdx.x;
    const int lane = tid & 63;
    const int wave = __builtin_amdgcn_readfirstlane(tid >> 6);
    const int half = lane >> 5;
    const int n = lane & 31;
    const int m0 = blockIdx.y * WROW;

    {
        const int nvec = p.Cin * (WROW / 4);
        for (int e = tid; e < nvec; e += 512) {
            const int ci = e / (WROW / 4), c4 = e % (WROW / 4);
            *reinterpret_cast<float4*>(wl + ci * WROW + 4 * c4) = *reinterpret_cast<const float4*>(p.wp + (int64_t)ci * p.Cout_pad + m0 + 4 * c4);
        }
    }
    __syncthreads();

    const int wstep = gridDim.x * 8;
    const unsigned xs = 8u * (unsigned)p.x.sC, xs2 = 8u * (unsigned)p.x2.sC;
    int b = 0, tin = 0, f = 0, t = 0;
    const char* xb = nullptr;
    const char* xb2 = nullptr;
    unsigned xo = 0, xo2 = 0;
    const float* sp = nullptr;
    float2 ring[U];
    float scr[SCALE ? U : 1];
    auto seek = [&](int tl) {
        b = tl / a.tps;
        tin = tl - b * a.tps;
        const int pos = tin * 64 + 2 * n;
        f = pos / p.T; t = pos - f * p.T;
        xb = reinterpret_cast<const char*>(p.x.p + (int64_t)b * p.x.sB);
        xb2 = p.x2.p ? reinterpret_cast<const char*>(p.x2.p + (int64_t)b * p.x2.sB) : xb;
        xo = 4u * (unsigned)(f * (int)p.x.sF + t + half * (int)p.x.sC);
        xo2 = p.x2.p ? 4u * (unsigned)(f * (int)p.x2.sF + t + half * (int)p.x2.sC) : xo;
        sp = SCALE ? p.in_scale + (int64_t)b * p.in_scale_ld + half : nullptr;
    };
    auto ld = [&](int s, int q) {
        if (s < a.nsteps1) ring[q] = *reinterpret_cast<const float2*>(xb + (xo + (unsigned)s * xs));
        else ring[q] = *reinterpret_cast<const float2*>(xb2 + (xo2 + (unsigned)(s - a.nsteps1) * xs2));
        if (SCALE) scr[q] = sp[2 * s];
    };
    for (int tl = blockIdx.x * 8 + wave; tl < a.ntiles; tl += wstep) {
        seek(tl);
#pragma unroll
        for (int q = 0; q < U; ++q) ld(q, q);
        f32x16 acc[MT][2];
#pragma unroll
        for (int i = 0; i < MT; ++i)
#pragma unroll
            for (int j = 0; j < 2; ++j)
#pragma unroll
                for (int r = 0; r < 16; ++r) acc[i][j][r] = 0.f;

        for (int s0 = 0; s0 < a.nsteps; s0 += U) {
            const bool more = s0 + U < a.nsteps;
            const float* wr0 = wl + (2 * s0 + half) * WROW + n;
#pragma unroll
            for (int q = 0; q < U; ++q) {
                float bx = ring[q].x, by = ring[q].y;
                if (SCALE) { bx *= scr[q]; by *= scr[q]; }
                if (more) ld(s0 + U + q, q);
                if (ACT) { bx = aid_gelu(bx); by = aid_gelu(by); }
#pragma unroll
                for (int i = 0; i < MT; ++i) {
                    const float aw = wr0[2 * q * WROW + 32 * i];
                    acc[i][0] = __builtin_amdgcn_mfma_f32_32x32x2f32(aw, bx, acc[i][0], 0, 0, 0);
                    acc[i][1] = __builtin_amdgcn_mfma_f32_32x32x2f32(aw, by, acc[i][1], 0, 0, 0);
                }
            }
        }

        const int be = b, tine = tin;
        char* yb = reinterpret_cast<char*>(p.y.p + (int64_t)b * p.y.sB);
        const char* rb = RES ? reinterpret_cast<const char*>(p.res.p + (int64_t)b * p.res.sB) : nullptr;
        const char* ab = EPI ? reinterpret_cast<const char*>(p.aux.p + (int64_t)b * p.aux.sB) : nullptr;
        const float* osb = p.out_scale ? p.out_scale + (int64_t)b * p.out_scale_ld : nullptr;
        const float* asb = EPI ? p.aux_scale + (int64_t)b * p.aux_scale_ld : nullptr;
        const unsigned ypos = 4u * (unsigned)(f * (int)p.y.sF + t);
        const unsigned rpos = RES ? 4u * (unsigned)(f * (int)p.res.sF + t) : 0u;
        const unsigned upos = EPI ? 4u * (unsigned)(f * (int)p.aux.sF + t) : 0u;
        float dsum[MT][4];
        int hv = half;
        asm volatile("" : "+v"(hv));
        const unsigned ys = 4u * (unsigned)p.y.sC, rs = 4u * (unsigned)p.res.sC, us = 4u * (unsigned)p.aux.sC;
        const int mb0 = m0 + 4 * hv;
        const unsigned yo = ypos + (unsigned)mb0 * ys;
        const unsigned ro = RES ? rpos + (unsigned)mb0 * rs : 0u;
        const unsigned uo = EPI ? upos + (unsigned)mb0 * us : 0u;
#pragma unroll
        for (int i = 0; i < MT; ++i) {
            const int mbase = mb0 + 32 * i;
#pragma unroll
            for (int q = 0; q < 4; ++q) dsum[i][q] = 0.f;
            constexpr int RB = 8;
#pragma unroll
            for (int r0 = 0; r0 < 16; r0 += RB) {
                float2 rv[RES ? RB : 1], uv[EPI ? RB : 1];
                float sv[RB], as[EPI ? RB : 1];
#pragma unroll
                for (int q = 0; q < RB; ++q) {
                    const int r = r0 + q;
                    const int dm = (r & 3) + 8 * (r >> 2);
                    if (RES) rv[q] = *reinterpret_cast<const float2*>(rb + (ro + (unsigned)(32 * i + dm) * rs));
                    sv[q] = osb ? osb[mbase + dm] : 1.f;
                    if (EPI) {
                        as[q] = asb[mbase + dm];
                        uv[q] = *reinterpret_cast<const float2*>(ab + (uo + (unsigned)(32 * i + dm) * us));
                    }
                }
#pragma unroll
                for (int q = 0; q < RB; ++q) {
                    const int r = r0 + q;
                    const int dm = (r & 3) + 8 * (r >> 2);
                    float y0 = acc[i][0][r] * sv[q], y1 = acc[i][1][r] * sv[q];
                    if (EPI) { y0 *= aid_dgelu(uv[q].x * as[q]); y1 *= aid_dgelu(uv[q].y * as[q]); }
                    if (RES) { y0 += p.res_scale * rv[q].x; y1 += p.res_scale * rv[q].y; }
                    y0 *= p.alpha; y1 *= p.alpha;
                    *reinterpret_cast<float2*>(yb + (yo + (unsigned)(32 * i + dm) * ys)) = make_float2(y0, y1);
                    if (EPI) dsum[i][r >> 2] += y0 * uv[q].x + y1 * uv[q].y;
                }
            }
        }
        if (EPI && p.dot_ws) {
            const int cpg = p.Cout >> 3;
            const int g = m0 / cpg + lane;
            float sacc = 0.f;
#pragma unroll
            for (int i = 0; i < MT; ++i)
#pragma unroll
                for (int q = 0; q < 4; ++q) {
                    float v = dsum[i][q];
#pragma unroll
                    for (int off = 16; off >= 1; off >>= 1) v += __shfl_xor(v, off, 32);
                    const float w = __shfl_xor(v, 32);
                    const float v0 = half ? w : v, v1 = half ? v : w;
                    const int c0 = m0 + 32 * i + 8 * q;
                    if (c0 / cpg == g) sacc += v0;
                    if ((c0 + 4) / cpg == g) sacc += v1;
                }
            if (lane < WROW / cpg && g < 8) p.dot_ws[((int64_t)be * 8 + g) * p.dot_n + tine] = (double)sacc;
        }
    }
}

template <int MT, int KMAX>
static int launch_c11rs(const aid_conv2d_params* p, hipStream_t st, const C11Plan& pl) {
    C11RDev a;
    a.p = *p;
    a.nsteps = p->Cin / 2;
    a.nsteps1 = pl.nsteps1;
    a.tps = pl.tps;
    a.ntiles = pl.ntiles;
    const dim3 grid((unsigned)pl.gx, (unsigned)pl.ny);
#define AID_C11RS(ACTv, SCv, EPIv, RESv) hipLaunchKernelGGL((conv11_rs_kernel<MT, KMAX, ACTv, SCv, EPIv, RESv>), grid, dim3(512), 0, st, a)
    switch (pl.key) {
        case 12: AID_C11RS(true, true, false, false); break;
        case 13: AID_C11RS(true, true, false, true); break;
        case 0:  AID_C11RS(false, false, false, false); break;
        case 1:  AID_C11RS(false, false, false, true); break;
        case 2:  AID_C11RS(false, false, true, false); break;
        case 3:  AID_C11RS(false, false, true, true); break;
        case 4:  AID_C11RS(false, true, false, false); break;
        case 5:  AID_C11RS(false, true, false, true); break;
        case 6:  AID_C11RS(false, true, true, false); break;
        default: aid_set_error("aid_conv2d: no conv11_rs_kernel instance for these options"); return AID_E_BADARG;
    }
#undef AID_C11RS
    AID_CHECK_LAUNCH();
    aid_note_kernel("conv11_rs_kernel");
    return AID_OK;
}

int aid_conv1x1_rs_try(const aid_conv2d_params* p, hipStream_t st) {
    if (!(p->KH == 1 && p->KW == 1)) return 0;
    const C11Plan pl = c11_rs_plan(c11_shape_of(*p));
    if (pl.family != C11_RS) return 0;
    if (!aid_view_aligned(p->x, 2) || !aid_view_aligned(p->y, 2) || (p->res.p && !aid_view_aligned(p->res, 2)) || (p->aux.p && !aid_view_aligned(p->aux, 2))) return 0;
    if (p->x2.p && !aid_view_aligned(p->x2, 2)) return 0;
    if (((uintptr_t)p->wp) & 15) return 0;
    auto fits = [&](const aid_view& v, int C) { return v.sC >= 0 && v.sF >= 0 && (int64_t)4 * ((int64_t)C * v.sC + (int64_t)p->F * v.sF + p->T) < (1LL << 32); };
    if (!fits(p->x, p->Cin) || !fits(p->y, p->Cout_pad) || (p->res.p && !fits(p->res, p->Cout_pad)) || (p->aux.p && !fits(p->aux, p->Cout_pad)) || (p->x2.p && !fits(p->x2, p->Cin))) return 0;
    if (p->dot_ws && p->dot_n != pl.slots) return 0;
    int rc;
    if (pl.MT == 3) rc = pl.KMAX == 128 ? launch_c11rs<3, 128>(p, st, pl) : launch_c11rs<3, 256>(p, st, pl);
    else            rc = launch_c11rs<2, 128>(p, st, pl);
    return rc == AID_OK ? 1 : rc;
}
```

audio_inpainting_diffusion_amd/csrc/aid_fin.h:

```cpp
#pragma once
#include "aid_common.h"

static __device__ __forceinline__ double aid_ld_agent(const double* q) {
    return __longlong_as_double((long long)__hip_atomic_load(reinterpret_cast<const unsigned long long*>(q), __ATOMIC_RELAXED, __HIP_MEMORY_SCOPE_AGENT));
}
static __device__ __forceinline__ void aid_st_agent(double* q, double v) {
    __hip_atomic_store(reinterpret_cast<unsigned long long*>(q), (unsigned long long)__double_as_longlong(v), __ATOMIC_RELAXED, __HIP_MEMORY_SCOPE_AGENT);
}
static __device__ __attribute__((noinline)) void aid_wino_fin(int mode, const double* ws, int nk, int b, int C, double n, const float* gamma, const float* mod, int64_t mod_ld,
                                                       float eps, float* scale, float* stats, double* sh, int tid, int nthr) {
    const int lane = tid & 63, wave = tid >> 6, nw = nthr >> 6;
    if (mode == 1) {
        for (int g = wave; g < 8; g += nw) {
            const double* w = ws + ((int64_t)(b * 8 + g) * nk) * 2;
            double s = 0.0, ss = 0.0;
            for (int i = lane; i < nk; i += 64) { s += aid_ld_agent(w + 2 * i); ss += aid_ld_agent(w + 2 * i + 1); }
#pragma unroll
            for (int off = 32; off >= 1; off >>= 1) { s += __shfl_xor(s, off, 64); ss += __shfl_xor(ss, off, 64); }
            if (lane == 0) { sh[2 * g] = s; sh[2 * g + 1] = ss; }
        }
        __syncthreads();
        const int cg = C >> 3;
        for (int c = tid; c < C; c += nthr) {
            const int g = c / cg;
            const double s = sh[2 * g], ss = sh[2 * g + 1];
            const double mean = s / n;
            double var = (ss - n * mean * mean) / (n - 1.0);
            if (var < 0.0) var = 0.0;
            const double inv = 1.0 / (sqrt(var) + (double)eps);
            const double m = mod ? (1.0 + (double)mod[(int64_t)b * mod_ld + c]) : 1.0;
            scale[(int64_t)b * C + c] = (float)((double)gamma[c] * m * inv);
            if (stats && c == g * cg) {
                stats[((int64_t)b * 8 + g) * 2 + 0] = (float)mean;
                stats[((int64_t)b * 8 + g) * 2 + 1] = (float)inv;
            }
        }
    } else {
        for (int g = wave; g < 8; g += nw) {
            const int i = b * 8 + g;
            const double* w = ws + (int64_t)i * nk;
            double d = 0.0;
            for (int k = lane; k < nk; k += 64) d += aid_ld_agent(w + k);
#pragma unroll
            for (int off = 32; off >= 1; off >>= 1) d += __shfl_xor(d, off, 64);
            if (lane == 0) {
                const double inv = (double)stats[2 * i + 1];
                const double sd = 1.0 / inv - (double)eps;
                scale[i] = (sd > 0.0) ? (float)(d * inv / ((n - 1.0) * sd)) : 0.f;
            }
        }
    }
}
```

audio_inpainting_diffusion_amd/network.py:

```python
from __future__ import annotations

import ctypes as C
import math
from typing import Callable, Dict, List, NamedTuple, Optional

import numpy as np
import torch
import torch.nn as nn

from . import _lib
from .cqt import CQTransform


class _Form(NamedTuple):
    code: int
    taps: int
    two_d: bool
    cols: Optional[Callable]


_FORMS = {0: _Form(0, 0, False, lambda T: T), 4: _Form(1, 30, False, lambda T: 6 * (T // 4)), 8: _Form(2, 50, False, lambda T: 10 * (T // 8)),
          45: _Form(3, 48, True, None), 85: _Form(4, 80, True, None)}


class _ConvPacks(NamedTuple):
    name: Optional[str]
    fwd: Dict[int, torch.Tensor]
    dgrad: Dict[int, torch.Tensor]


RSQRT2 = 1.0 / math.sqrt(2.0)
SQRT2 = math.sqrt(2.0)
_CUBIC = (-0.01171875, -0.03515625, 0.11328125, 0.43359375, 0.43359375, 0.11328125, -0.03515625, -0.01171875)


def _kaiming_uniform(shape, fan_in, scale):
    return (torch.rand(*shape) * 2 - 1) * math.sqrt(3.0 / fan_in) * scale


class _Weight(nn.Module):
    def __init__(self, shape, fan_in, scale, bias_len=0):
        super().__init__()
        self.weight = nn.Parameter(_kaiming_uniform(shape, fan_in, scale))
        if bias_len:
            self.bias = nn.Parameter(torch.zeros(bias_len))


class _Gamma(nn.Module):
    def __init__(self, n):
        super().__init__()
        self.gamma = nn.Parameter(torch.ones(1, n, 1, 1))


class _Kernel(nn.Module):
    def __init__(self):
        super().__init__()
        self.register_buffer("kernel", torch.tensor(_CUBIC, dtype=torch.float32))


class _Embedding(nn.Module):

    def __init__(self, emb_dim, rff_dim=32):
        super().__init__()
        self.RFF_freq = nn.Parameter(16 * torch.randn([1, rff_dim]), requires_grad=False)
        s = math.sqrt(1 / 3)
        self.MLP = nn.ModuleList([_Weight([128, 2 * rff_dim], 2 * rff_dim, s, 128), _Weight([256, 128], 128, s, 256),
                                  _Weight([emb_dim, 256], 256, s, emb_dim)])


class _RelPos(nn.Module):

    def __init__(self, num_buckets, max_distance, heads):
        super().__init__()
        self.num_buckets, self.max_distance = int(num_buckets), int(max_distance)
        self.relative_attention_bias = _Weight([num_buckets, heads], heads, 1.0)

    def buckets(self, T: int) -> torch.Tensor:
        nb = self.num_buckets // 2
        pos = torch.arange(T, dtype=torch.long)
        rel = pos[None, :] - pos[:, None]
        ret = (rel >= 0).to(torch.long) * nb
        n = torch.abs(rel)
        max_exact = nb // 2
        val_if_large = max_exact + (torch.log(n.float() / max_exact) / math.log(self.max_distance / max_exact) * (nb - max_exact)).long()
        val_if_large = torch.min(val_if_large, torch.full_like(val_if_large, nb - 1))
        return ret + torch.where(n < max_exact, n, val_if_large)

    def bias_table(self, T: int) -> torch.Tensor:
        w = self.relative_attention_bias.weight.detach().float()
        return w[self.buckets(T).to(w.device)].permute(2, 0, 1).contiguous()


class _FreqEnc(nn.Module):

    def __init__(self, f_dim, N):
        super().__init__()
        self.RFF_freq = nn.Parameter(16 * torch.randn([1, N]), requires_grad=False)
        table = 2 * math.pi * torch.arange(f_dim)[None, None, :] * self.RFF_freq.unsqueeze(-1)
        self.embeddings = nn.Parameter(torch.cat([torch.sin(table), torch.cos(table)], dim=1), requires_grad=False)


class _Attn(nn.Module):

    def __init__(self, nin, heads, fdim, bias_qkv=False, rel_pos=None):
        super().__init__()
        s = math.sqrt(1 / 3)
        n = heads * fdim
        self.qk = _Weight([2 * n, n, 1], n, s, bias_len=2 * n if bias_qkv else 0)
        self.proj_in = _Weight([heads, nin, 1, 1], nin, s)
        self.proj_out = _Weight([nin, heads, 1, 1], heads, s)
        if rel_pos is not None:
            self.rel_pos = _RelPos(*rel_pos, heads)


class _ResBlock(nn.Module):

    def __init__(self, dim, dim_out, num_dils, kernel_size, emb_dim, proj_place="before", attention=False, heads=8, fdim=0,
                 bias_qkv=False, rel_pos=None):
        super().__init__()
        self.dim, self.dim_out, self.num_dils, self.ks, self.proj_place = dim, dim_out, num_dils, tuple(kernel_size), proj_place
        self.has_attn, self.heads, self.fdim = attention, heads, fdim
        s, z = math.sqrt(1 / 3), 1e-7
        N = dim_out if proj_place == "before" else dim
        self.N = N
        if proj_place != "before" and N != dim_out:
            self.proj_out = _Weight([dim_out, N, 1, 1], N, s)
        if dim != dim_out:
            self.res_conv = _Weight([dim_out, dim, 1, 1], dim, s)
        if dim != N:
            self.proj_in = _Weight([N, dim, 1, 1], dim, s)
        kh, kw = self.ks
        self.H = nn.ModuleList([_Weight([N, N, kh, kw], N * kh * kw, s) for _ in range(num_dils)])
        self.affine = nn.ModuleList([_Weight([N, emb_dim], emb_dim, s, N) for _ in range(num_dils)])
        self.gate = nn.ModuleList([_Weight([N, emb_dim], emb_dim, z, N) for _ in range(num_dils)])
        self.norm = nn.ModuleList([_Gamma(N) for _ in range(num_dils)])
        if attention:
            self.norm2 = _Gamma(N)
            self.affine2 = _Weight([N, emb_dim], emb_dim, s, N)
            self.gate2 = _Weight([N, emb_dim], emb_dim, z, N)
            self.attn_block = _Attn(N, heads, fdim, bias_qkv, rel_pos)


from .plan import Plan as _Plan


class _Builder:
    def __init__(self, net, B, device, train=False):
        self.net, self.B, self.device = net, B, device
        self.train = bool(train)
        self.S_of = {}
        self.mod = self.dmod = None
        self.pgrad = None
        self.params = None
        self.plan = _Plan()
        self.nbytes = 0
        self.lane = 0
        self.use_lanes = not self.train and bool(getattr(net, "plan_lanes", True))
        self._stats_ws = {}
        self._keep = []
        self.whole_batch = True
        self.bwd = []
        self._stat_src = {}
        self._nb_src = {}
        self._g_last = {}
        self._in_bwd = False
        self.bplan = None
        self.gmap = {}
        self.gstate = {}
        self.scratch = {}
        self.galias = {}

    def G(self, t, _peek=False):
        st = t.untyped_storage()
        g = self.gmap.get(st.data_ptr())
        if g is None:
            g = self.gmap[st.data_ptr()] = torch.zeros(st.nbytes() // 4, device=self.device, dtype=torch.float32)
            self.nbytes += g.numel() * 4
        gv = g.as_strided(t.size(), t.stride(), t.storage_offset())
        if self.galias and not _peek:
            self._materialise(g.untyped_storage().data_ptr())
        return gv

    def _defer_copy(self, src, dst, c):
        if not self.net.fold_grad_copies or self.train or not self._in_bwd:
            self.add2_raw(src, None, dst, c, 0.0)
            return
        key = dst.untyped_storage().data_ptr()
        self._materialise(key)
        self.galias.setdefault(key, []).append((self._vkey(dst), dst, src, float(c)))

    def _materialise(self, storage_ptr=None):
        for key in ([storage_ptr] if storage_ptr is not None else list(self.galias)):
            for _vk, dst, src, c in self.galias.pop(key, ()):
                self.add2_raw(src, None, dst, c, 0.0)

    def Gsrc(self, t):
        gv = self.G(t, _peek=True)
        key = gv.untyped_storage().data_ptr()
        pend = self.galias.get(key)
        if pend and len(pend) == 1 and pend[0][0] == self._vkey(gv):
            _vk, _dst, src, c = self.galias.pop(key)[0]
            return src, c
        return self.G(t), 1.0

    def _gacc(self, t) -> bool:
        st = t.untyped_storage()
        key = st.data_ptr()
        state = self.gstate.get(key)
        if state is None:
            whole = t.is_contiguous() and t.numel() * 4 == st.nbytes()
            self.gstate[key] = "full" if whole else "zero"
            return not whole
        return True

    def _scratch(self, shape):
        key = (self.lane,) + tuple(shape)
        t = self.scratch.get(key)
        if t is None:
            t = self.scratch[key] = self.buf(*[d for d in tuple(shape) if not isinstance(d, str)])
        return t

    def _split_ws(self, nbytes):
        key = (self.lane, "w4r_split")
        t = self.scratch.get(key)
        if t is None or t.numel() * 4 < nbytes:
            if t is not None:
                self._keep.append(t)
            t = self.scratch[key] = torch.zeros(max(nbytes, 4096 + 336 * 98304) // 4, device=self.device, dtype=torch.float32)
            self.nbytes += t.numel() * 4
        if not any(t is z for z in self.plan.zero_on_fail):
            self.plan.zero_on_fail.append(t)
        return t

    @property
    def stats_ws(self):
        t = self._stats_ws.get(self.lane)
        if t is None:
            t = self._stats_ws[self.lane] = torch.empty(self.B * 8 * _lib.AID_STATS_SPLIT * 2, device=self.device, dtype=torch.float64)
            self.nbytes += t.numel() * 8
        return t

    def on_lane(self, lane):
        bd = self

        class _L:
            def __enter__(self_):
                self_.prev, bd.lane = bd.lane, (lane if bd.use_lanes else 0)

            def __exit__(self_, *a):
                bd.lane = self_.prev
        return _L()

    def _add(self, name, params, *tensors, **kw):
        self.plan.lane = self.lane
        return self.plan.add(name, params, *tensors, **kw)

    def _reg_bwd(self, fn):
        self.bwd.append((self.lane, fn))

    def finish_backward(self):
        fwd_plan, self.plan = self.plan, _Plan()
        self._in_bwd = True
        self._stat_src.clear()
        self._nb_src.clear()
        self._g_last.clear()
        for lane, emit in reversed(self.bwd):
            self.lane = lane
            emit()
        self.lane = 0
        self._materialise()
        self._in_bwd = False
        self.bplan, self.plan = self.plan, fwd_plan
        return self.bplan

    def buf(self, *shape):
        t = torch.empty(*shape, device=self.device, dtype=torch.float32)
        self.nbytes += t.numel() * 4
        return t

    @staticmethod
    def _vkey(t):
        return (t.data_ptr(), tuple(t.shape), tuple(t.stride()))

    def _wrote(self, t):
        d = self._nb_src if self._in_bwd else self._stat_src
        if not d or t is None:
            return
        lo = t.data_ptr()
        hi = lo + 4 * (1 + sum((n - 1) * st for n, st in zip(t.shape, t.stride())))
        for k in [k for k, v in d.items() if not (v[2] <= lo or hi <= k[0])]:
            del d[k]

    def stats(self, x, gamma, mod, scale, stats=None, gname=None):
        B, Cc, F, T = x.shape
        src = None if self._in_bwd else self._stat_src.pop(self._vkey(x), None)
        ws, ws_n = self.stats_ws, 0
        if src is not None:
            cp, ws_n = src[0], src[1]
            ws = torch.empty(B * 8 * ws_n * 2, device=self.device, dtype=torch.float64)
            self.nbytes += ws.numel() * 8
            cp.stat_ws, cp.stat_n = ws.data_ptr(), ws_n
            src[3].also_writes(ws)
            if self.net.fuse_fin and self._fin_wanted(cp.B, src[4]) and _lib.lib().aid_conv2d_fin_supported(cp.B, cp.Cin, cp.Cout, cp.F, cp.T, cp.dilF, cp.x_wino):
                cnt = self._fin_count(src[3].lane)
                cp.fin_mode, cp.fin_count, cp.fin_gamma, cp.fin_eps = 1, cnt.data_ptr(), gamma.data_ptr(), 1e-7
                cp.fin_mod, cp.fin_mod_ld = _lib.ptr(mod), (0 if mod is None else mod.stride(0))
                cp.fin_scale, cp.fin_stats = scale.data_ptr(), _lib.ptr(stats)
                src[3].also_writes(scale, stats, cnt)
                src[3].also_reads(gamma, mod)
                self.plan.keep.extend(t for t in (ws, gamma, mod, scale, stats, cnt) if t is not None)
                self._stats_train_hook(scale, gamma, mod, gname, stats, B, Cc)
                return
        p = _lib.GroupStatsParams(_lib.view4(x), B, Cc, F, T, 8, gamma.data_ptr(), _lib.ptr(mod),
                                  0 if mod is None else mod.stride(0), 1e-7, scale.data_ptr(), _lib.ptr(stats),
                                  ws.data_ptr(), ws_n)
        self._add("aid_group_stats", p, x, gamma, mod, scale, stats, ws, writes=(scale, stats) + (() if src is not None else (ws,)))
        self._stats_train_hook(scale, gamma, mod, gname, stats, B, Cc)

    @staticmethod
    def _fin_wanted(B, form):
        return not _FORMS[form].two_d or B <= 2

    def _fin_count(self, lane):
        key = (lane, "fin_count")
        t = self.scratch.get(key)
        if t is None:
            t = self.scratch[key] = torch.zeros(self.B, device=self.device, dtype=torch.int32)
        if not any(t is z for z in self.plan.zero_on_fail):
            self.plan.zero_on_fail.append(t)
        return t

    def _stats_train_hook(self, scale, gamma, mod, gname, stats, B, Cc):
        if self.train and gname is not None:
            def bw():
                S = self.S_of.pop(scale.data_ptr(), None)
                if S is None:
                    return
                dm = self.dmod_like(mod)
                sp = _lib.ScaleBwdParams(S.data_ptr(), S.stride(0), scale.data_ptr(), scale.stride(0), gamma.data_ptr(), _lib.ptr(mod),
                                         0 if mod is None else mod.stride(0), stats.data_ptr(), self.pgrad[gname].data_ptr(),
                                         _lib.ptr(dm), 0 if dm is None else dm.stride(0), B, Cc, 8, 1)
                self._add("aid_scale_bwd", sp, S, scale, gamma, mod, stats, dm, writes=(self.pgrad[gname], dm))
            self._reg_bwd(bw)

    def dmod_like(self, view):
        if view is None:
            return None
        off = (view.data_ptr() - self.mod.data_ptr()) // 4
        assert 0 <= off < self.mod.shape[1] and view.stride(0) == self.mod.stride(0)
        return self.dmod[:, off:off + view.shape[1]]

    def _train_conv(self, x, gy, gd, rec, cin, cout, kh, kw, dil, in_scale, act, out_scale, alpha):
        B, _, F, T = gy.shape
        K = kh * kw
        wu, wname = rec.fwd.get(4), rec.name
        wino = bool(self.net.wgrad_wino and (kh, kw) == (5, 3) and T % 16 == 0 and cin >= 32 and cout >= 32
                    and (out_scale is None or wu is not None))
        xin, isc = x, in_scale
        if wino:
            G6 = _FORMS[4].cols(T)
            xin = self._scratch(("hww", B, cin, F, G6))
            sp = _lib.ScaleActParams(_lib.view4(x), _lib.view4(xin), _lib.ptr(in_scale) if act else None,
                                     in_scale.stride(0) if (act and in_scale is not None) else 0, B, cin, F, T, 1 if act else 0, 1)
            self._add("aid_scale_act", sp, x, xin, in_scale, writes=(xin,))
            if act:
                isc = None
            gyw = self._scratch(("gyw", B, cout, F, G6))
            self._add("aid_wino_gy", _lib.WinoGyParams(_lib.view4(gy), _lib.view4(gyw), B, cout, F, T), gy, gyw, writes=(gyw,))
            gop = gyw
        else:
            gop = gy
            if act:
                xin = self._scratch(("hw",) + tuple(x.shape))
                sp = _lib.ScaleActParams(_lib.view4(x), _lib.view4(xin), in_scale.data_ptr(), in_scale.stride(0), B, cin, F, T, 1, 0)
                self._add("aid_scale_act", sp, x, xin, in_scale, writes=(xin,))
                isc = None
        tiles = int(_lib.lib().aid_conv2d_wgrad_tiles(cin, cout, kh, kw, int(wino)))
        S = max(1, min(F, 256 // (tiles * B)))
        KP = _FORMS[4].taps if wino else K
        P = self._scratch(("P", B * S * cout * cin * KP))
        wp = _lib.WgradParams(_lib.view4(gop), _lib.view4(xin), P.data_ptr(), B, cin, cout, F, T, kh, kw, dil, S, alpha, int(wino))
        self._add("aid_conv2d_wgrad", wp, gop, xin, P, flops=2 * B * F * T * cin * cout * K, writes=(P,))
        W = self.params[wname]
        dg = self.dmod_like(out_scale)
        rp = _lib.WgradReduceParams(P.data_ptr(), W.data_ptr(), _lib.ptr(out_scale), 0 if out_scale is None else out_scale.stride(0),
                                    _lib.ptr(isc), 0 if isc is None else isc.stride(0), self.pgrad[wname].data_ptr(), _lib.ptr(dg),
                                    0 if dg is None else dg.stride(0), B, S, cout, cin, K, 1, int(wino),
                                    _lib.ptr(wu) if wino else None, wu.shape[1] if (wino and wu is not None) else 0,
                                    wu.shape[2] if (wino and wu is not None) else 0)
        self._add("aid_wgrad_reduce", rp, P, W, out_scale, isc, dg, wu, writes=(self.pgrad[wname], dg))
        if in_scale is not None and gd is not None:
            Sb = self.buf(B, cin)
            cp = _lib.ChannelDotParams(_lib.view4(gd), _lib.view4(x), Sb.data_ptr(), Sb.stride(0), B, cin, F, T)
            self._add("aid_channel_dot", cp, gd, x, Sb, writes=(Sb,))
            self.S_of[in_scale.data_ptr()] = Sb

    def _conv_raw(self, x, y, wp, cin, cout, kh, kw, dil, in_scale, act, out_scale, res, res_scale, alpha, epi=0,
                  aux=None, aux_scale=None, wu=None, form=0, dot=None, x2=None, fin_stats=None):
        B, _, F, T = y.shape
        fm = _FORMS[form]
        p = _lib.Conv2dParams()
        nxi = fm.taps if fm.two_d else 0
        if nxi:
            npos = self._w2d_positions(form, B, F, T, dil)
            assert x.dim() == 1 and x.numel() == nxi * cin * npos and x2 is None and in_scale is None and not act
            p.x = _lib.View(x.data_ptr(), 0, 0, 0)
        else:
            assert x.shape[1] + (0 if x2 is None else x2.shape[1]) == cin and y.shape[1] == cout and x.shape[0] == B and x.shape[2] == F
            assert x.shape[3] == fm.cols(T)
            p.x = _lib.view4(x)
        p.y, p.res, p.aux = _lib.view4(y), _lib.view4(res), _lib.view4(aux)
        p.wp = wp.data_ptr()
        p.in_scale, p.in_scale_ld = _lib.ptr(in_scale), (0 if in_scale is None else in_scale.stride(0))
        p.out_scale, p.out_scale_ld = _lib.ptr(out_scale), (0 if out_scale is None else out_scale.stride(0))
        p.aux_scale, p.aux_scale_ld = _lib.ptr(aux_scale), (0 if aux_scale is None else aux_scale.stride(0))
        p.B, p.Cin, p.Cout, p.F, p.T = B, cin, cout, F, T
        p.Cin_pad, p.Cout_pad = wp.shape[1], wp.shape[2]
        p.KH, p.KW, p.dilF, p.act, p.epi = kh, kw, dil, act, epi
        p.alpha, p.res_scale = alpha, res_scale
        p.wp_wino = _lib.ptr(wu)
        p.wino_taps = 0 if wu is None else wu.shape[0]
        p.x_wino = fm.code
        if dot is not None:
            p.dot_ws, p.dot_n = dot[0].data_ptr(), dot[1]
        cnt = None
        if fin_stats is not None:
            cnt = self._fin_count(self.lane)
            p.fin_mode, p.fin_count, p.fin_eps, p.fin_stats = 2, cnt.data_ptr(), 1e-7, fin_stats.data_ptr()
            p.fin_scale = dot[0].data_ptr() + 8 * B * 8 * dot[1]
        if x2 is not None:
            p.x2, p.Cin1 = _lib.view4(x2), x.shape[1]
        ws = None
        if F == 1 and kh == 1 and epi == 0:
            ws = self._scratch(("ws", 8 * B * cout * T))
            p.ws, p.ws_bytes = ws.data_ptr(), ws.numel() * 4
        elif nxi:
            ws = self._scratch(("m45", nxi * cout * npos))
            p.ws, p.ws_bytes = ws.data_ptr(), ws.numel() * 4
        elif form == 4 and B == 1 and self.whole_batch:
            need = int(_lib.lib().aid_conv2d_wino_split_ws_bytes(B, cin, cout, F, T, dil))
            if need:
                ws = self._split_ws(need)
                p.ws, p.ws_bytes = ws.data_ptr(), ws.numel() * 4
        assert wp.shape[0] == kh * kw and (wu is None or (wu.shape[0] == _FORMS[form or 4].taps and wu.shape[1:] == wp.shape[1:]))
        nb = 4 * (B * F * T * (cin + cout * (1 + (res is not None) + (aux is not None))) + cin * cout * kh * kw)
        dws = None if dot is None else dot[0]
        if nxi:
            mxi = nxi // 2 if (form == 85 and cin <= 128 and 10 * (-(-npos // 64)) * (-(-cout // 128)) >= 768) else nxi
            self._add("aid_conv2d_wino2d_gemm", p, x, wu, ws, flops=2 * B * F * T * cin * cout * kh * kw, nbytes=4 * npos * (nxi * cin + mxi * cout), writes=(ws,))
            op = self._add("aid_conv2d_wino2d_output", p, ws, y, res, out_scale, aux, aux_scale, dws, fin_stats, cnt,
                           nbytes=4 * (mxi * npos * cout + B * F * T * cout * (1 + (res is not None) + (aux is not None))), writes=(y, dws, cnt))
        else:
            op = self._add("aid_conv2d", p, x, x2, y, res, wp, in_scale, out_scale, aux, aux_scale, wu, ws, dws, fin_stats, cnt, flops=2 * B * F * T * cin * cout * kh * kw,
                           nbytes=nb, writes=(y, ws, dws, cnt))
        self._wrote(y)
        if not self._in_bwd and form and epi == 0 and dot is None and self.net.epilogue_stats:
            n = int(_lib.lib().aid_conv2d_stat_partials(B, cin, cout, F, T, dil, fm.code))
            if n:
                hi = y.data_ptr() + 4 * (1 + sum((m - 1) * st for m, st in zip(y.shape, y.stride())))
                self._stat_src[self._vkey(y)] = (p, n, hi, op, form)

    def _dot_ws(self, n):
        key = (self.lane, "dot", n)
        t = self.scratch.get(key)
        if t is None:
            t = self.scratch[key] = torch.zeros(self.B * 8 * (n + 1), device=self.device, dtype=torch.float64)
            self.nbytes += t.numel() * 8
        return t

    @staticmethod
    def _w2d_positions(form, B, F, T, dil):
        n = int(_lib.lib().aid_conv2d_wino2d_positions(B, F, T, dil))
        return n // 2 if form == 85 else n

    def _form(self, rec, dgrad, cin, cout, F, T, dil):
        packs = rec.dgrad if dgrad else rec.fwd
        if 4 not in packs:
            return 0
        L, net, wf, fb = _lib.lib(), self.net, tuple(self.net.wino_forms), int(self.net.form_batch or self.B)
        forced2d = wf in ((45,), (85,), (45, 85))
        if 45 in packs and (45 in wf or 85 in wf) and L.aid_conv2d_wino2d_supported(cin, cout, F, T, dil) and (forced2d or (
                min(cin, cout) >= net.w2d_min_channels and (T <= net.w2d_force_max_T or L.aid_conv2d_wino2d_wanted(fb, cin, cout, F, T, dil))
                and (cout % 128 == 0 or T <= net.w2d_c96_max_T))):
            if 85 in packs and 85 in wf and T % 32 == 0 and (45 not in wf or cout % 128 != 0 or int(L.aid_conv2d_wino2d_tform(fb, cin, cout, F, T, dil)) == 8):
                return 85
            if 45 in wf:
                return 45
        form = int(L.aid_conv2d_wino_form(fb, cin, cout, F, T, dil))
        if form == 8 and (8 not in packs or 8 not in wf):
            form = 4
        elif form == 4 and 4 not in wf and 8 in packs and L.aid_conv2d_wino8_supported(cin, cout, F, T, dil):
            form = 8
        return 0 if form == 4 and not ((4 in wf or forced2d) and L.aid_conv2d_wino_input_ok(self.B, cin, cout, F, T, dil)) else form

    def _wino_scratch(self, tag, form, B, C, F, T, dil):
        fm = _FORMS[form]
        return self._scratch((tag + "45", fm.taps * C * self._w2d_positions(form, B, F, T, dil)) if fm.two_d else (tag, B, C, F, fm.cols(T)))

    @staticmethod
    def _sa_out(t):
        return _lib.View(t.data_ptr(), 0, 0, 0) if t.dim() == 1 else _lib.view4(t)

    def conv(self, x, y, w, cin, cout, kh=1, kw=1, dil=1, in_scale=None, act=0, out_scale=None, res=None,
             res_scale=1.0, alpha=1.0, norm_stats=None, res_nograd=False):
        rec = w if isinstance(w, _ConvPacks) else _ConvPacks(None, {0: w}, {})
        B, _, F, T = x.shape
        if act and kh > 1:
            xw = self._form(rec, False, cin, cout, F, T, dil)
            hbuf = self._wino_scratch("h", xw, B, cin, F, T, dil)
            sp = _lib.ScaleActParams(_lib.view4(x), self._sa_out(hbuf), in_scale.data_ptr(), in_scale.stride(0), B, cin, F, T, 1, _FORMS[xw].code, dil)
            self._add("aid_scale_act", sp, x, hbuf, in_scale, writes=(hbuf,))
            self._conv_raw(hbuf, y, rec.fwd[0], cin, cout, kh, kw, dil, None, 0, out_scale, res, res_scale, alpha, wu=rec.fwd.get(xw or 4), form=xw)
        else:
            self._conv_raw(x, y, rec.fwd[0], cin, cout, kh, kw, dil, in_scale, act, out_scale, res, res_scale, alpha)
        if not rec.dgrad:
            return

        def bw():
            fused_res = (norm_stats is not None) and (res is x)
            gy, gmul = self.Gsrc(y) if (kh > 1 and out_scale is not None and norm_stats is not None and fused_res and not self.train) else (self.G(y), 1.0)
            if res is not None and not fused_res and not res_nograd:
                gr = self.G(res)
                if self._gacc(res):
                    self.add2_raw(gr, gy, gr, 1.0, alpha * res_scale)
                else:
                    self.add2_raw(gy, None, gr, alpha * res_scale, 0.0)
            gin, gsc, gw = gy, out_scale, 0
            if kh > 1 and out_scale is not None:
                gw = self._form(rec, True, cout, cin, gy.shape[2], gy.shape[3], dil) if norm_stats is not None else 0
                gin = self._wino_scratch("g", gw, gy.shape[0], cout, gy.shape[2], gy.shape[3], dil)
                nb = self._nb_src.pop(self._vkey(gy), None) if (gw and self.net.fuse_norm_bwd_wino and gmul == 1.0) else None
                if nb is not None and nb[1] > self._g_last.get(gin.data_ptr(), -1) and nb[3].lane == self.lane:
                    nb[0].wout, nb[0].wscale, nb[0].wscale_ld = self._sa_out(gin), out_scale.data_ptr(), out_scale.stride(0)
                    nb[0].wform, nb[0].wdil = _FORMS[gw].code, dil
                    self.plan.keep.extend((gin, out_scale))
                    nb[3].also_writes(gin)
                else:
                    sp = _lib.ScaleActParams(_lib.view4(gy), self._sa_out(gin), out_scale.data_ptr(), out_scale.stride(0), gy.shape[0],
                                             cout, gy.shape[2], gy.shape[3], 0, _FORMS[gw].code, dil, 0.0 if gmul == 1.0 else gmul)
                    self._add("aid_scale_act", sp, gy, gin, out_scale, writes=(gin,))
                self._g_last[gin.data_ptr()] = len(self.plan.ops)
                gsc = None
            if norm_stats is not None:
                gd = self._scratch(x.shape)
                nd = 0
                if act and kh == 5 and gsc is None and 4 in rec.dgrad:
                    nd = int(_lib.lib().aid_conv2d_dot_partials(B, cout, cin, F, T, dil, _FORMS[gw].code))
                elif act and kh == 1 and kw == 1 and self.net.fuse_dot_1x1:
                    nd = int(_lib.lib().aid_conv2d_dot_partials_1x1(B, cout, cin, F, T))
                dws = self._dot_ws(nd) if nd else self.stats_ws
                fin = bool(nd and kh == 5 and gw and self.net.fuse_fin and self._fin_wanted(B, gw)
                           and _lib.lib().aid_conv2d_fin_supported(B, cout, cin, F, T, dil, _FORMS[gw].code))
                self._conv_raw(gin, gd, rec.dgrad[0], cout, cin, kh, kw, dil, gsc, 0, in_scale, None, 1.0, alpha,
                               epi=1 if act else 0, aux=x if act else None, aux_scale=in_scale if act else None, wu=rec.dgrad.get(gw or 4), form=gw,
                               dot=(dws, nd) if nd else None, fin_stats=norm_stats if fin else None)
                if not nd:
                    dp = _lib.GroupDotParams(_lib.view4(gd), _lib.view4(x), B, cin, F, T, 8, self.stats_ws.data_ptr())
                    self._add("aid_group_dot", dp, gd, x, self.stats_ws, writes=(self.stats_ws,))
                if self.train and rec.name is not None:
                    self._train_conv(x, gy, gd, rec, cin, cout, kh, kw, dil, in_scale, act, out_scale, alpha)
                npar = _lib.NormBwdParams(_lib.view4(gd), _lib.view4(x), _lib.view4(gy if fused_res else None), _lib.view4(self.G(x)),
                                          B, cin, F, T, 8, norm_stats.data_ptr(), dws.data_ptr(), 1e-7,
                                          alpha * res_scale * gmul, 1 if self._gacc(x) else 0, nd)
                npar.coef_ready = 1 if fin else 0
                gxv = self.G(x)
                nop = self._add("aid_norm_bwd", npar, gd, x, gy, norm_stats, dws, gxv, writes=(gxv,))
                self._wrote(gxv)
                if npar.accumulate == 0 and x.shape[3] % 16 == 0:
                    hi = gxv.data_ptr() + 4 * (1 + sum((m - 1) * st for m, st in zip(gxv.shape, gxv.stride())))
                    self._nb_src[self._vkey(gxv)] = (npar, len(self.plan.ops) - 1, hi, nop)
            else:
                gx = self.G(x)
                self._conv_raw(gin, gx, rec.dgrad[0], cout, cin, kh, kw, dil, gsc, 0, in_scale, gx if self._gacc(x) else None, 1.0 / alpha, alpha,
                               epi=1 if act else 0, aux=x if act else None, aux_scale=in_scale if act else None)
                if self.train and rec.name is not None:
                    assert in_scale is None, "a scaled conv input without its statistics buffer has no parameter-gradient path"
                    self._train_conv(x, gy, None, rec, cin, cout, kh, kw, dil, None, act, out_scale, alpha)
        self._reg_bwd(bw)


    def pair_dgrad(self, xin, x0, yout, wpair, n, cout):
        def bw():
            g1, g2, gx = self.G(x0), self.G(yout), self.G(xin)
            self._conv_raw(g1, gx, wpair, 2 * n, cout, 1, 1, 1, None, 0, None, gx if self._gacc(xin) else None, 1.0, 1.0, x2=g2)
        self._reg_bwd(bw)

    def res_grad(self, res, y, c):
        def bw():
            gy = self.G(y)
            if self._gacc(res):
                gr = self.G(res)
                self.add2_raw(gr, gy, gr, 1.0, c)
            else:
                self._defer_copy(gy, self.G(res, _peek=True), c)
        self._reg_bwd(bw)

    def add2_raw(self, u, v, y, a, b):
        B, Cc, F, T = u.shape
        p = _lib.Add2Params(_lib.view4(u), _lib.view4(v), _lib.view4(y), B, Cc, F, T, a, b)
        self._add("aid_add2", p, u, v, y, writes=(y,))
        self._wrote(y)

    def add2(self, u, v, y, a, b):
        self.add2_raw(u, v, y, a, b)

        def bw():
            gy = self.G(y)
            for tt, c in ((u, a), (v, b)):
                if self._gacc(tt):
                    gt = self.G(tt)
                    self.add2_raw(gt, gy, gt, 1.0, c)
                else:
                    self._defer_copy(gy, self.G(tt, _peek=True), c)
        self._reg_bwd(bw)

    def copy(self, u, y):
        self.add2_raw(u, None, y, 1.0, 0.0)

        def bw():
            gy, gu = self.G(y), self.G(u)
            if self._gacc(u):
                self.add2_raw(gu, gy, gu, 1.0, 1.0)
            else:
                self.add2_raw(gy, None, gu, 1.0, 0.0)
        self._reg_bwd(bw)

    def _resample_raw(self, x, y, up, adjoint=0, accumulate=0):
        B, Cc, F, T = x.shape
        p = _lib.ResampleParams(_lib.view4(x), _lib.view4(y), B, Cc, F, T, int(up), int(adjoint), int(accumulate))
        self._add("aid_resample", p, x, y, writes=(y,))
        self._wrote(y)

    def resample(self, x, y, up):
        self._resample_raw(x, y, up)
        self._reg_bwd(lambda: self._resample_raw(self.G(y), self.G(x), up, adjoint=1, accumulate=1 if self._gacc(x) else 0))

    def attention(self, qk, v, out, heads, F, T, bias=None, relpos=None):
        B = v.shape[0]
        probs = self.buf(B, heads, T, T)
        scale = float(F) ** -0.5
        p = _lib.AttentionParams(qk.data_ptr(), v.data_ptr(), out.data_ptr(), probs.data_ptr(), B, heads, F, T, scale, _lib.ptr(bias))
        self._add("aid_time_attention", p, qk, v, out, probs, bias, flops=4 * B * heads * T * T * F, writes=(out, probs))
        self._wrote(out)

        def bw():
            gq, gv, go = self.G(qk), self.G(v), self.G(out)
            assert gq.is_contiguous() and gv.is_contiguous() and go.is_contiguous()
            self._gacc(qk)
            dsws = self._scratch(("ds", B, heads, T, T))
            bp = _lib.AttentionBwdParams(qk.data_ptr(), v.data_ptr(), probs.data_ptr(), go.data_ptr(), gq.data_ptr(), gv.data_ptr(),
                                         B, heads, F, T, scale, 1 if self._gacc(v) else 0, dsws.data_ptr())
            self._add("aid_time_attention_bwd", bp, qk, v, probs, go, gq, gv, dsws, flops=10 * B * heads * T * T * F, writes=(gq, gv, dsws))
            self._wrote(gq)
            self._wrote(gv)
            if self.train and relpos is not None:
                bucket, wname = relpos
                dW = self.pgrad[wname]
                rp = _lib.RelposBwdParams(dsws.data_ptr(), bucket.data_ptr(), dW.data_ptr(), B, heads, T, dW.shape[0], 1)
                self._add("aid_relpos_bwd", rp, dsws, bucket, dW, writes=(dW,))
        self._reg_bwd(bw)

    def bias_grad(self, y, wname):
        def bw():
            gy = self.G(y)
            B, Cc, F, T = gy.shape
            ones = self.scratch.get(("ones", T))
            if ones is None:
                ones = self.scratch[("ones", T)] = torch.ones(max(T, 4), device=self.device, dtype=torch.float32)
            S = self.buf(B, Cc)
            ov = _lib.View(ones.data_ptr(), 0, 0, 0)
            cp = _lib.ChannelDotParams(_lib.view4(gy), ov, S.data_ptr(), S.stride(0), B, Cc, F, T)
            self._add("aid_channel_dot", cp, gy, ones, S, writes=(S,))
            dW = self.pgrad[wname]
            rp = _lib.WgradReduceParams(S.data_ptr(), self.params[wname].data_ptr(), None, 0, None, 0, dW.data_ptr(), None, 0,
                                        B, 1, Cc, 1, 1, 1, 0, None, 0, 0)
            self._add("aid_wgrad_reduce", rp, S, dW, writes=(dW,))
        self._reg_bwd(bw)


class Unet_CQT_oct_with_attention(nn.Module):

    def __init__(self, args, device):
        super().__init__()
        self.args = args
        net = args.network if hasattr(args, "network") else args
        self.depth = self.num_octs = int(net.cqt.num_octs)
        self.bins_per_oct = int(net.cqt.bins_per_oct)
        self.emb_dim = int(net.emb_dim)
        has_attn = any(int(v) for v in net.attention_layers)
        if not net.use_norm:
            raise NotImplementedError("use_norm=False is not built (every shipped configuration normalises)")
        if net.bottleneck_type != "res_dil_convs":
            raise NotImplementedError("bottleneck type not implemented")
        self.heads = int(net.attention_dict.num_heads)
        self.Ns = [int(v) for v in net.Ns]
        self.num_dils = [int(v) for v in net.num_dils]
        self.attention_layers = [int(v) for v in net.attention_layers]
        self.num_bottleneck_layers = int(net.num_bottleneck_layers)
        self.device = torch.device(device)
        win = ("kaiser", float(net.cqt.beta)) if net.cqt.window == "kaiser" else net.cqt.window
        self.CQTransform = CQTransform(self.num_octs, self.bins_per_oct, mode="oct", window=win,
                                       fs=args.exp.sample_rate, audio_len=args.exp.audio_len, dtype=torch.float32,
                                       device=self.device, rules=net.cqt.get("rules") if hasattr(net.cqt, "get") else None)
        n, E, bpo, H = self.num_octs, self.emb_dim, self.bins_per_oct, self.heads
        self.embedding = _Embedding(E)
        ad = net.attention_dict
        akw = dict(heads=H, bias_qkv=bool(ad.bias_qkv),
                   rel_pos=(int(ad.rel_pos_num_buckets), int(ad.rel_pos_max_distance)) if ad.use_rel_pos else None)
        self.use_fencoding = bool(net.use_fencoding)
        self.n_fenc = 32
        if self.use_fencoding:
            self.freq_encodings = nn.ModuleList([_FreqEnc(bpo, self.n_fenc) for _ in range(n)])
        Nin = 2 * self.n_fenc + 2 if self.use_fencoding else 2
        self.Nin = Nin
        self.downsamplerT, self.upsamplerT = _Kernel(), _Kernel()
        self.downs, self.middle, self.ups = nn.ModuleList(), nn.ModuleList(), nn.ModuleList()
        s = math.sqrt(1 / 3)
        for i in range(n):
            dim_in = self.Ns[i] if i == 0 else self.Ns[i - 1]
            dim_out = self.Ns[i]
            self.downs.append(nn.ModuleList([
                _ResBlock(Nin, dim_in, 1, (1, 1), E),
                _Weight([dim_out, 2, 5, 3], 2 * 15, s),
                _ResBlock(dim_in, dim_out, self.num_dils[i], (5, 3), E, attention=bool(self.attention_layers[i]),
                          fdim=(i + 1) * bpo, **akw)]))
        for _ in range(self.num_bottleneck_layers):
            self.middle.append(nn.ModuleList([
                _ResBlock(self.Ns[-1], 2, 1, (1, 1), E, proj_place="after"),
                _ResBlock(self.Ns[-1], self.Ns[-1], self.num_dils[-1], (5, 3), E, attention=bool(self.attention_layers[-1]),
                          fdim=n * bpo, **akw)]))
        for i in range(n - 1, -1, -1):
            dim_in = self.Ns[i] * 2
            dim_out = self.Ns[i] if i == 0 else self.Ns[i - 1]
            self.ups.append(nn.ModuleList([
                _ResBlock(dim_out, 2, 1, (1, 1), E, proj_place="after"),
                _ResBlock(dim_in, dim_out, self.num_dils[i], (5, 3), E, attention=bool(self.attention_layers[i]),
                          fdim=(i + 1) * bpo, **akw)]))
        self._packed: Dict[str, torch.Tensor] = {}
        self._conv_packs: Dict[str, _ConvPacks] = {}
        self._packed_ver = None
        self._states: Dict[tuple, dict] = {}
        self._mod_layout = None
        self.to(self.device)

    def _param_version(self):
        return tuple(p._version for p in self.parameters()) + (id(next(self.parameters())),)

    def _resblocks(self):
        for i, m in enumerate(self.downs):
            yield f"downs.{i}.0.", m[0]
            yield f"downs.{i}.2.", m[2]
        for i, m in enumerate(self.middle):
            yield f"middle.{i}.0.", m[0]
            yield f"middle.{i}.1.", m[1]
        for i, m in enumerate(self.ups):
            yield f"ups.{i}.0.", m[0]
            yield f"ups.{i}.1.", m[1]

    @torch.no_grad()
    def prepare(self, force=False):
# ... 763 lines not shown
```

include/aid_kernels.h:

```cpp
#ifndef AID_KERNELS_H
#define AID_KERNELS_H

#include <stdint.h>

#ifdef __cplusplus
extern "C" {
#endif

#define AID_OK 0
#define AID_E_BADARG (-1)
#define AID_E_LAUNCH (-2)

#define AID_ABI_VERSION 14
int aid_abi_version(void);
const char* aid_last_error(void);
const char* aid_last_kernel(void);

typedef struct {
    float* p;
    int64_t sB, sC, sF;
} aid_view;

#define AID_STATS_SPLIT 32
typedef struct {
    aid_view x;
    int B, C, F, T, groups;
    const float* gamma;
    const float* mod;
    int64_t mod_ld;
    float eps;
    float* scale;
    float* stats;
    double* ws;
    int ws_n;
} aid_group_stats_params;
int aid_group_stats(const aid_group_stats_params* p, void* stream);

typedef struct {
    aid_view x, y, res, aux;
    const float* wp;
    const float* in_scale;   int64_t in_scale_ld;
    const float* out_scale;  int64_t out_scale_ld;
    const float* aux_scale;  int64_t aux_scale_ld;
    int B, Cin, Cout, F, T;
    int Cin_pad, Cout_pad;
    int KH, KW, dilF;
    int act, epi;
    float alpha, res_scale;
    const float* wp_wino;
    int wino_taps;
    int x_wino;
    float* ws; int64_t ws_bytes;
    double* dot_ws; int dot_n;
    double* stat_ws; int stat_n;
    aid_view x2; int Cin1;
    int fin_mode;
    unsigned* fin_count;
    const float* fin_gamma;
    const float* fin_mod; int64_t fin_mod_ld;
    float fin_eps;
    float* fin_scale;
    float* fin_stats;
} aid_conv2d_params;
int aid_conv2d(const aid_conv2d_params* p, void* stream);
int aid_conv2d_dot_partials_1x1(int B, int Cin, int Cout, int F, int T);
int aid_conv2d_x2_supported(int Cin, int Cin1, int Cout, int F, int T);
int aid_conv2d_wino_input_supported(int Cin, int Cout, int T);
int aid_conv2d_wino_input_ok(int B, int Cin, int Cout, int F, int T, int dilF);
int aid_conv2d_wino_form(int B, int Cin, int Cout, int F, int T, int dilF);
int aid_conv2d_wino8_supported(int Cin, int Cout, int F, int T, int dilF);
#define AID_CONV2D_SPLIT_FLAG_BYTES 4096
int64_t aid_conv2d_wino_split_ws_bytes(int B, int Cin, int Cout, int F, int T, int dilF);
int aid_conv2d_fin_supported(int B, int Cin, int Cout, int F, int T, int dilF, int x_wino);
int aid_conv2d_dot_partials(int B, int Cin, int Cout, int F, int T, int dilF, int x_wino);
int aid_conv2d_stat_partials(int B, int Cin, int Cout, int F, int T, int dilF, int x_wino);
int aid_conv2d_wino2d_supported(int Cin, int Cout, int F, int T, int dilF);
int64_t aid_conv2d_wino2d_positions(int B, int F, int T, int dilF);
int aid_conv2d_wino2d_wanted(int B, int Cin, int Cout, int F, int T, int dilF);
int aid_conv2d_wino2d_tform(int B, int Cin, int Cout, int F, int T, int dilF);
void aid_conv2d_pack_dims(int Cin, int Cout, int* Cin_pad, int* Cout_pad);

typedef struct {
    const float* U; const float* V; float* M;
    int nxi, Cin, Cout, Cin_pad, Cout_pad;
    int64_t N;
    int variant;
} aid_wino2d_gemm_params;
int aid_wino2d_gemm(const aid_wino2d_gemm_params* p, void* stream);
int aid_conv2d_wino2d_gemm(const aid_conv2d_params* p, void* stream);
int aid_conv2d_wino2d_output(const aid_conv2d_params* p, void* stream);
int aid_wino2d_set_split(int pieces);

typedef struct {
    aid_view x, y;
    int B, C, F, T;
    int up, adjoint;
    int accumulate;
} aid_resample_params;
int aid_resample(const aid_resample_params* p, void* stream);

typedef struct {
    const float* qk; const float* v; float* out; float* probs;
    int B, H, F, T;
    float scale;
    const float* bias;
} aid_attention_params;
int aid_time_attention(const aid_attention_params* p, void* stream);

typedef struct {
    const float* sigma;
    const float* rff_freq;
    const float* w0; const float* b0;
    const float* w1; const float* b1;
    const float* w2; const float* b2;
    float* emb;
    int B, rff, h0, h1, E;
} aid_embed_params;
int aid_embed(const aid_embed_params* p, void* stream);

typedef struct {
    const float* emb; const float* W; const float* bias; float* mod;
    int B, E, N;
} aid_modulation_params;
int aid_modulation(const aid_modulation_params* p, void* stream);

typedef struct {
    int n_oct, bins;
    const int* rc;
    const int* Lg;
    const int* goff;
    const float* g;
    const int* T_oct;
    const float* twiddle;
    int Tmax;
} aid_cqt_tables;

#define AID_CQT_MAX_OCT 12
typedef struct {
    aid_cqt_tables tab;
    int T_host[AID_CQT_MAX_OCT];
    aid_view oct[AID_CQT_MAX_OCT];
    const float* spec;
    float* band_ws;
    const float* in_scale;
    int B, Lh;
    int unnormalized;
} aid_cqt_params;
int aid_cqt_analysis(const aid_cqt_params* p, void* stream);
int aid_cqt_synthesis(const aid_cqt_params* p, void* stream);

typedef struct {
    const float* band_ws;
    const int* kfirst; const int* kcount;
    const int* rc; const int* Lg; const int* goff; const int* woff; const int* Tk;
    const float* gdM;
    const float* X;
    const float* cskip; const float* cout;
    const float* hpf;
    float* Y;
    int B, Lh; int64_t ws_per_b;
    const float* band_scale;
} aid_cqt_gather_params;
int aid_cqt_gather(const aid_cqt_gather_params* p, void* stream);

typedef struct {
    const float* in; float* out; const float* twiddle;
    int B, N, R, Ns;
    int in_mode, out_mode;
    float sign, out_scale;
} aid_fft_pass_params;
int aid_fft_pass(const aid_fft_pass_params* p, void* stream);

typedef struct {
    const float* x; const float* y; float* out;
    const float* a; const float* b;
    int B; int64_t L;
    float a_host, b_host;
} aid_axpby_params;
int aid_axpby(const aid_axpby_params* p, void* stream);

typedef struct {
    const float* x; const float* xhat; const float* yobs; const float* smask; int64_t smask_sB;
    const float* x0; const float* d0;
    const float* t; const float* h;
    float* xnext; float* dout; float* xh_out;
    int B; int64_t L; int mode;
    float t_host, h_host;
} aid_score_step_params;
int aid_score_step(const aid_score_step_params* p, void* stream);

typedef struct {
    aid_view u, v;
    int B, C, F, T, groups;
    double* ws;
} aid_group_dot_params;
int aid_group_dot(const aid_group_dot_params* p, void* stream);

typedef struct {
    aid_view gd, x, gy, out;
    int B, C, F, T, groups;
    const float* stats;
    const double* ws;
    float eps, a;
    int accumulate;
    int ws_n;
    aid_view wout;
    const float* wscale; int64_t wscale_ld;
    int wform;
    int coef_ready;
    int wdil;
} aid_norm_bwd_params;
int aid_norm_bwd(const aid_norm_bwd_params* p, void* stream);

typedef struct {
    const float* qk; const float* v; const float* probs; const float* gout;
    float* gqk; float* gv;
    int B, H, F, T;
    float scale;
    int accumulate_gv;
    float* ws;
} aid_attention_bwd_params;
int aid_time_attention_bwd(const aid_attention_bwd_params* p, void* stream);

typedef struct {
    const float* xhat; const float* y; const float* mask; int64_t mask_sB;
    float* g; float* norm;
    int B; int64_t L;
    int norm_type;
    float beta;
} aid_guidance_seed_params;
int aid_guidance_seed(const aid_guidance_seed_params* p, void* stream);

typedef struct {
    const float* xhat; const float* g; float* out; float* step_out; float* s_out;
    int B; int64_t L;
    float coef, inv_sqrt_len, eps;
} aid_guidance_step_params;
int aid_guidance_step(const aid_guidance_step_params* p, void* stream);

typedef struct { float* out; int64_t ld; int B, n; float v[8]; } aid_set_rows_params;
int aid_set_rows(const aid_set_rows_params* p, void* stream);

typedef struct { const float* x; float* out; int B; int64_t L; } aid_row_norm_params;
int aid_row_norm(const aid_row_norm_params* p, void* stream);

typedef struct {
    const float* x; float* y; const float* kernel;
    int64_t x_ld, y_ld;
    int64_t L, Lout;
    int B, orig_freq, new_freq, width, K;
} aid_resample_poly_params;
int aid_resample_poly(const aid_resample_poly_params* p, void* stream);

typedef struct {
    const float* x; float* frames; float* out;
    const float* window; const float* twiddle; const float* inv_env;
    const float* mask; int64_t mask_sB; int64_t mask_ld;
    const float* add1; const float* add2; float c0;
    int B; int64_t L; int64_t Lp;
    int n_fft, hop, n_frames, adjoint;
} aid_stft_params;
int aid_stft_frames(const aid_stft_params* p, void* stream);
int aid_stft_ola(const aid_stft_params* p, void* stream);

typedef struct {
    aid_view x, y;
    const float* scale; int64_t scale_ld;
    int B, C, F, T, act;
    int wino;
    int dilF;
    float mul;
} aid_scale_act_params;
int aid_scale_act(const aid_scale_act_params* p, void* stream);

typedef struct {
    aid_view u, v, y;
    int B, C, F, T;
    float a, b;
} aid_add2_params;
int aid_add2(const aid_add2_params* p, void* stream);

typedef struct {
    aid_view gy, x;
    float* P;
    int B, Cin, Cout, F, T, KH, KW, dilF;
    int S;
    float alpha;
    int wino;
} aid_conv2d_wgrad_params;
int aid_conv2d_wgrad(const aid_conv2d_wgrad_params* p, void* stream);
int aid_conv2d_wgrad_tiles(int Cin, int Cout, int KH, int KW, int wino);

typedef struct { aid_view gy, out; int B, C, F, T; } aid_wino_gy_params;
int aid_wino_gy(const aid_wino_gy_params* p, void* stream);

typedef struct {
    const float* w;
    float* wp; float* wpT; float* wpw; float* wpwT;
    int Cout, Cin, KH, KW;
    int Cin_pad, Cout_pad, Cin_padT, Cout_padT;
    float* wpw8; float* wpw8T;
    float* wpw2; float* wpw2T;
    float* wpw3; float* wpw3T;
} aid_pack_conv_weight_params;
int aid_pack_conv_weight(const aid_pack_conv_weight_params* p, void* stream);

typedef struct {
    const float* P; const float* W;
    const float* gate; int64_t gate_ld;
    const float* in_scale; int64_t in_scale_ld;
    float* dW; float* dgate; int64_t dgate_ld;
    int B, S, Cout, Cin, K, accumulate;
    int wino;
    const float* Uw;
    int Cin_pad, Cout_pad;
} aid_wgrad_reduce_params;
int aid_wgrad_reduce(const aid_wgrad_reduce_params* p, void* stream);

typedef struct {
    aid_view u, v;
    float* out; int64_t out_ld;
    int B, C, F, T;
} aid_channel_dot_params;
int aid_channel_dot(const aid_channel_dot_params* p, void* stream);

typedef struct {
    const float* dS;
    const int* bucket;
    float* dW;
    int B, H, T, num_buckets, accumulate;
} aid_relpos_bwd_params;
int aid_relpos_bwd(const aid_relpos_bwd_params* p, void* stream);

typedef struct {
    const float* S; int64_t S_ld;
    const float* scale; int64_t scale_ld;
    const float* gamma; const float* mod; int64_t mod_ld;
    const float* stats;
    float* dgamma; float* dmod; int64_t dmod_ld;
    int B, C, groups, accumulate;
} aid_scale_bwd_params;
int aid_scale_bwd(const aid_scale_bwd_params* p, void* stream);

typedef struct {
    const float* dmod; const float* emb; const float* W;
    float* dW; float* dbias; float* demb;
    int B, E, N, accumulate;
    float* part; int64_t part_floats;
} aid_modulation_bwd_params;
int aid_modulation_bwd(const aid_modulation_bwd_params* p, void* stream);

typedef struct {
    aid_embed_params fwd;
    const float* demb;
    float* dw0; float* db0; float* dw1; float* db1; float* dw2; float* db2;
    int accumulate;
} aid_embed_bwd_params;
int aid_embed_bwd(const aid_embed_bwd_params* p, void* stream);

typedef struct {
    float* param; const float* grad; float* m; float* v;
    const float* gscale;
    int64_t n;
    float lr, beta1, beta2, eps, bias1, bias2_sqrt;
} aid_adam_params;
int aid_adam(const aid_adam_params* p, void* stream);

typedef struct { float* dst; const float* src; int64_t n; float rate; } aid_ema_params;
// ... 11 lines not shown
```

Before: 63.75 denoiser evaluations (one segment each) per second, whole job.

## Fuse group-norm statistics and finalize into 1x1 conv epilogues

Extends the 1x1 convolution kernels (row-shared and DMA families) to accumulate per-group sum and sum-of-squares of their outputs in the epilogue and write partials to a stat workspace. Optionally the last block finalizes the group norm scale via an atomic counter, as the 5x3 Winograd kernels already do. This removes the separate statistics pass over the activation that follows 1x1 layers feeding a norm. The cost is extra registers and reductions in the epilogue, a narrower set of eligible plan shapes, and a grid-wide completion counter.

After: 63.85 denoiser evaluations (one segment each) per second, whole job, median of 2. Within noise of the previous version (+0.2%).

```diff
diff --git a/audio_inpainting_diffusion_amd/_lib.py b/audio_inpainting_diffusion_amd/_lib.py
--- a/audio_inpainting_diffusion_amd/_lib.py
+++ b/audio_inpainting_diffusion_amd/_lib.py
@@ -347,7 +347,7 @@
            "aid_time_attention", "aid_embed", "aid_modulation", "aid_cqt_analysis", "aid_cqt_synthesis",
            "aid_cqt_gather", "aid_axpby", "aid_score_step", "aid_add2", "aid_group_dot", "aid_norm_bwd",
            "aid_time_attention_bwd", "aid_guidance_seed", "aid_guidance_step", "aid_set_rows", "aid_row_norm", "aid_scale_act", "aid_fft_pass",
-           "aid_stft_frames", "aid_stft_ola", "aid_resample_poly", "aid_conv2d_wino_input_supported", "aid_conv2d_dot_partials", "aid_conv2d_x2_supported", "aid_conv2d_dot_partials_1x1", "aid_conv2d_wino_input_ok", "aid_conv2d_wino_form", "aid_conv2d_wino8_supported", "aid_conv2d_wino_split_ws_bytes", "aid_conv2d_fin_supported",
+           "aid_stft_frames", "aid_stft_ola", "aid_resample_poly", "aid_conv2d_wino_input_supported", "aid_conv2d_dot_partials", "aid_conv2d_x2_supported", "aid_conv2d_dot_partials_1x1", "aid_conv2d_stat_partials_1x1", "aid_conv2d_fin_supported_1x1", "aid_conv2d_wino_input_ok", "aid_conv2d_wino_form", "aid_conv2d_wino8_supported", "aid_conv2d_wino_split_ws_bytes", "aid_conv2d_fin_supported",
            "aid_conv2d_wgrad", "aid_wgrad_reduce", "aid_channel_dot", "aid_relpos_bwd", "aid_scale_bwd", "aid_modulation_bwd", "aid_embed_bwd",
            "aid_adam", "aid_ema", "aid_sumsq", "aid_wino2d_gemm", "aid_wino2d_set_split", "aid_conv2d_wino2d_gemm", "aid_conv2d_wino2d_output", "aid_conv2d_wino2d_supported", "aid_conv2d_wino2d_positions", "aid_conv2d_wino2d_wanted", "aid_conv2d_wino2d_tform"]
 
@@ -377,6 +377,10 @@
         L.aid_conv2d_x2_supported.restype = C.c_int
         L.aid_conv2d_dot_partials_1x1.argtypes = [C.c_int] * 5
         L.aid_conv2d_dot_partials_1x1.restype = C.c_int
+        L.aid_conv2d_stat_partials_1x1.argtypes = [C.c_int] * 5
+        L.aid_conv2d_stat_partials_1x1.restype = C.c_int
+        L.aid_conv2d_fin_supported_1x1.argtypes = [C.c_int] * 5
+        L.aid_conv2d_fin_supported_1x1.restype = C.c_int
         L.aid_conv2d_wino_input_ok.argtypes = [C.c_int] * 6
         L.aid_conv2d_wino_input_ok.restype = C.c_int
         L.aid_conv2d_wino8_supported.argtypes = [C.c_int] * 5
@@ -402,7 +406,7 @@
         L.aid_wino2d_set_split.argtypes = [C.c_int]
         L.aid_wino2d_set_split.restype = C.c_int
         for name in EXPORTS[3:]:
-            if name not in ("aid_conv2d_pack_dims", "aid_conv2d_wino_input_supported", "aid_conv2d_dot_partials", "aid_conv2d_x2_supported", "aid_conv2d_dot_partials_1x1", "aid_conv2d_wino_input_ok", "aid_conv2d_wino_form", "aid_conv2d_wino8_supported", "aid_conv2d_wino_split_ws_bytes", "aid_conv2d_fin_supported",
+            if name not in ("aid_conv2d_pack_dims", "aid_conv2d_wino_input_supported", "aid_conv2d_dot_partials", "aid_conv2d_x2_supported", "aid_conv2d_dot_partials_1x1", "aid_conv2d_stat_partials_1x1", "aid_conv2d_fin_supported_1x1", "aid_conv2d_wino_input_ok", "aid_conv2d_wino_form", "aid_conv2d_wino8_supported", "aid_conv2d_wino_split_ws_bytes", "aid_conv2d_fin_supported",
                             "aid_conv2d_stat_partials", "aid_conv2d_wgrad_tiles", "aid_conv2d_wino2d_supported", "aid_conv2d_wino2d_positions", "aid_conv2d_wino2d_wanted", "aid_conv2d_wino2d_tform", "aid_wino2d_set_split"):
                 getattr(L, name).argtypes = [C.c_void_p, C.c_void_p]
                 getattr(L, name).restype = C.c_int
diff --git a/audio_inpainting_diffusion_amd/csrc/aid_conv.hip b/audio_inpainting_diffusion_amd/csrc/aid_conv.hip
--- a/audio_inpainting_diffusion_amd/csrc/aid_conv.hip
+++ b/audio_inpainting_diffusion_amd/csrc/aid_conv.hip
@@ -463,6 +463,20 @@
     return c11_plan(s).slots;
 }
 
+extern "C" int aid_conv2d_stat_partials_1x1(int B, int Cin, int Cout, int F, int T) {
+    C11Shape s = c11_query_shape(B, Cin, Cout, F, T);
+    s.stat = true;
+    const C11Plan pl = c11_plan(s);
+    return pl.ok ? pl.slots : 0;
+}
+
+extern "C" int aid_conv2d_fin_supported_1x1(int B, int Cin, int Cout, int F, int T) {
+    C11Shape s = c11_query_shape(B, Cin, Cout, F, T);
+    s.stat = true;
+    const C11Plan pl = c11_plan(s);
+    return (pl.ok && pl.slots > 0) ? (pl.family == C11_RS ? 2 : 1) : 0;
+}
+
 extern "C" int aid_conv2d_x2_supported(int Cin, int Cin1, int Cout, int F, int T) {
     C11Shape s = c11_query_shape(1, Cin, Cout, F, T);
     s.x2 = true; s.Cin1 = Cin1;
@@ -482,12 +496,18 @@
     AID_REQUIRE(p->epi == 0 || (p->epi == 1 && p->aux.p && p->aux_scale), "aid_conv2d: epi=1 needs aux + aux_scale");
     AID_REQUIRE((int64_t)p->B * p->in_scale_ld < (1LL << 31), "aid_conv2d: in_scale too large");
     AID_REQUIRE(!p->x_wino || (p->KH == 5 && p->KW == 3 && p->wp_wino), "aid_conv2d: x_wino is a 5x3 Winograd-path input layout");
-    AID_REQUIRE(!p->fin_mode || (p->x_wino && p->KH == 5 && p->KW == 3), "aid_conv2d: fin_mode is an option of the row-shared 5x3 Winograd kernels (aid_conv2d_fin_supported)");
+    AID_REQUIRE(!p->fin_mode || (p->x_wino && p->KH == 5 && p->KW == 3) || (p->KH == 1 && p->KW == 1 && p->fin_mode == 1 && p->stat_ws),
+                "aid_conv2d: fin_mode is an option of the row-shared 5x3 Winograd kernels (aid_conv2d_fin_supported) and, as 1 with stat_ws, of 1x1 layers (aid_conv2d_fin_supported_1x1)");
     if (p->x_wino == 3 || p->x_wino == 4) return aid_conv53_wino2d(p, st);
     if (p->x2.p) {
+        AID_REQUIRE(!p->stat_ws, "aid_conv2d: stat_ws is not an option of the two-tensor K axis");
         AID_REQUIRE(p->KH == 1 && p->KW == 1 && !p->in_scale && p->act == 0 && p->Cin1 > 0 && p->Cin1 < p->Cin && (p->Cin1 % 16) == 0 && ((p->Cin - p->Cin1) % 16) == 0,
                     "aid_conv2d: x2 is an option of plain 1x1 convolutions with both K segments multiples of 16");
         return conv1x1_dispatch(p, st, "aid_conv2d: x2 given but the layer is not eligible for the 1x1 kernels that take it");
+    }
+    if (p->stat_ws && p->KH == 1 && p->KW == 1) {
+        AID_REQUIRE(!p->dot_ws && p->epi == 0 && p->act == 0 && p->stat_n > 0, "aid_conv2d: stat_ws on a 1x1 layer is an option of the plain forward epilogue (epi = 0, act = 0, no dot_ws)");
+        return conv1x1_dispatch(p, st, "aid_conv2d: stat_ws given but the 1x1 layer is not eligible (aid_conv2d_stat_partials_1x1)");
     }
     if (p->stat_ws) {
         AID_REQUIRE(!p->dot_ws && p->epi == 0 && p->x_wino, "aid_conv2d: stat_ws is an option of the forward epilogue on Winograd-domain input");
diff --git a/audio_inpainting_diffusion_amd/csrc/aid_conv1x1_dma.hip b/audio_inpainting_diffusion_amd/csrc/aid_conv1x1_dma.hip
--- a/audio_inpainting_diffusion_amd/csrc/aid_conv1x1_dma.hip
+++ b/audio_inpainting_diffusion_amd/csrc/aid_conv1x1_dma.hip
@@ -1,6 +1,8 @@
 #include "aid_common.h"
 #include "aid_mfma_dma.h"
 #include "aid_conv1x1_plan.h"
+#include "aid_conv1x1_stat.h"
+#include "aid_fin.h"
 #include <type_traits>
 
 int aid_conv_splitk_reduce(const aid_conv2d_params* p, const float* ws, int splits, hipStream_t st);
@@ -14,6 +16,7 @@
     int nch1;
     int splits, cps;
     float* ws;
+    int fin_total;
 };
 
 __device__ float4 g_aid_zero_page_c11[16];
@@ -183,7 +186,7 @@
     const int f = rowinfo[2 * rr + 1];
     const int t = t0 + tt;
     const bool live = !(b < 0 || t >= p.T);
-    if (!live && !p.dot_ws) return;
+    if (!live && !p.dot_ws && !p.stat_ws) return;
     if (live && a.splits > 1) {
         const int64_t ft = (int64_t)p.F * p.T;
         float* wsb = a.ws + (((int64_t)blockIdx.y * p.B + b) * p.Cout) * ft + (int64_t)f * p.T + t;
@@ -202,10 +205,11 @@
     const int64_t rbase = p.res.p ? ((int64_t)b * p.res.sB + (int64_t)f * p.res.sF + t) : 0;
     const int64_t abase = p.aux.p ? ((int64_t)b * p.aux.sB + (int64_t)f * p.aux.sF + t) : 0;
     float dsum[MT][4];
+    float qsum[MT][4];
 #pragma unroll
     for (int i = 0; i < MT; ++i)
 #pragma unroll
-        for (int q = 0; q < 4; ++q) dsum[i][q] = 0.f;
+        for (int q = 0; q < 4; ++q) { dsum[i][q] = 0.f; qsum[i][q] = 0.f; }
 #pragma unroll
     for (int i = 0; i < MT; ++i) {
         if (!live) break;
@@ -238,6 +242,7 @@
                 y0 *= p.alpha; y1 *= p.alpha;
                 *reinterpret_cast<float2*>(p.y.p + ybase + (int64_t)m * p.y.sC) = make_float2(y0, y1);
                 if (p.dot_ws) dsum[i][r0 >> 2] += y0 * uv[q].x + y1 * uv[q].y;
+                if (p.stat_ws) { dsum[i][r0 >> 2] += y0 + y1; qsum[i][r0 >> 2] += y0 * y0 + y1 * y1; }
             }
         }
     }
@@ -275,6 +280,45 @@
             p.dot_ws[((int64_t)bt * 8 + grp) * p.dot_n + ptile] = (double)sacc;
         }
     }
+    if (p.stat_ws) {
+        double* red = reinterpret_cast<double*>(sbuf0);
+        const int bt = rowinfo[0];
+        c11_stat_cpg<MT>(p.Cout >> 3, [&](auto cpgc) {
+            constexpr int CPG = decltype(cpgc)::value;
+            constexpr int NS = c11_stat_slots(MT, CPG);
+            double v1, v2;
+            const int slot = c11_stat_wave<MT, CPG>(dsum, qsum, lane, v1, v2);
+            if ((lane & (64 / NS - 1)) == 0) { red[(wave * 8 + slot) * 2] = v1; red[(wave * 8 + slot) * 2 + 1] = v2; }
+            __syncthreads();
+            if constexpr (M_BLK % CPG == 0) {
+                const int grp = m0 / CPG + tid;
+                if (tid < M_BLK / CPG && grp < 8) {
+                    double a1 = 0.0, a2 = 0.0;
+                    for (int w = 0; w < NW; ++w) {
+                        const int k = tid - ((w / WGN) * 32 * MT) / CPG;
+                        if (k >= 0 && k < NS) { a1 += red[(w * 8 + k) * 2]; a2 += red[(w * 8 + k) * 2 + 1]; }
+                    }
+                    const int ptile = ((row0 - bt * p.F) >> a.rows_log2) * a.tiles_t + tile_t;
+                    double* o = p.stat_ws + (((int64_t)bt * 8 + grp) * p.stat_n + ptile) * 2;
+                    if (p.fin_mode) { aid_st_agent(o, a1); aid_st_agent(o + 1, a2); }
+                    else { o[0] = a1; o[1] = a2; }
+                }
+            }
+        });
+        if (p.fin_mode) {
+            asm volatile("s_waitcnt vmcnt(0)" ::: "memory");
+            __syncthreads();
+            int* shi = reinterpret_cast<int*>(sbuf1);
+            if (tid == 0) shi[0] = (__hip_atomic_fetch_add(p.fin_count + bt, 1u, __ATOMIC_RELAXED, __HIP_MEMORY_SCOPE_AGENT) == (unsigned)(a.fin_total - 1)) ? 1 : 0;
+            __syncthreads();
+            if (shi[0]) {
+                const double n = (double)(p.Cout >> 3) * (double)p.F * (double)p.T;
+                aid_wino_fin(1, p.stat_ws, p.stat_n, bt, p.Cout, n, p.fin_gamma, p.fin_mod, p.fin_mod_ld, p.fin_eps, p.fin_scale, p.fin_stats,
+                             reinterpret_cast<double*>(sbuf1) + 2, tid, NTHREADS);
+                if (tid == 0) __hip_atomic_store(p.fin_count + bt, 0u, __ATOMIC_RELAXED, __HIP_MEMORY_SCOPE_AGENT);
+            }
+        }
+    }
 }
 
 template <int MT, int WGM, int WGN, int RMAX, int KC, int MINW>
@@ -300,6 +344,7 @@
     a.cps = pl.kps / KC;
     a.splits = aid_cdiv(a.nchunks, a.cps);
     a.ws = (float*)p->ws;
+    a.fin_total = pl.slots * pl.ny;
     hipLaunchKernelGGL((conv11_dma_kernel<MT, WGM, WGN, RMAX, KC, MINW>), dim3((unsigned)(8 * a.per_xcd), (unsigned)a.splits), dim3(64 * WGM * WGN), 0, st, a);
     AID_CHECK_LAUNCH();
     aid_note_kernel(a.splits > 1 ? "conv11_dma_kernel+splitk" : "conv11_dma_kernel");
@@ -369,6 +414,7 @@
     if ((int64_t)4 * 16 * p->x.sC >= (1LL << 31)) return 0;
     if (p->x2.p && (!aid_view_aligned(p->x2, 4) || (int64_t)4 * 16 * p->x2.sC >= (1LL << 31))) return 0;
     if (p->dot_ws && p->dot_n != pl.slots) return 0;
+    { const int rc = c11_stat_check(p, pl.slots, pl.MT); if (rc != 1) return rc; }
     if (pl.S > 1 && !aid_conv_splitk_scratch_ok(p, pl.S)) {
         s.ws = false;
         pl = c11_dma_plan(s);
diff --git a/audio_inpainting_diffusion_amd/csrc/aid_conv1x1_plan.h b/audio_inpainting_diffusion_amd/csrc/aid_conv1x1_plan.h
--- a/audio_inpainting_diffusion_amd/csrc/aid_conv1x1_plan.h
+++ b/audio_inpainting_diffusion_amd/csrc/aid_conv1x1_plan.h
@@ -10,6 +10,7 @@
     bool in_scale, res, x2, dot;
     bool ws;
     int64_t ws_bytes;
+    bool stat;
 };
 
 struct C11Plan {
@@ -60,6 +61,8 @@
 
 static inline C11Plan c11_none() { C11Plan pl = {}; pl.ok = true; return pl; }
 
+static inline bool c11_stat_excluded(const C11Shape& s) { return s.stat && (s.epi != 0 || s.x2 || s.dot || s.act); }
+
 static inline C11Plan c11_rs_plan(const C11Shape& s) {
     C11Plan pl = c11_none();
     if (!c11_rs_enabled() || s.ws || (s.act && !s.in_scale) || s.Cout != s.Cout_pad) return pl;
@@ -73,7 +76,7 @@
     if (s.x2 && ((s.Cin1 % 2) || s.Cin1 <= 0 || s.Cin1 >= s.Cin || s.in_scale || s.act)) return pl;
     const int key = (s.act ? 8 : 0) | (s.in_scale ? 4 : 0) | (s.epi == 1 ? 2 : 0) | (s.res ? 1 : 0);
     if (!(key <= 6 || key == 12 || key == 13)) return pl;
-    if (s.dot && s.epi != 1) return pl;
+    if ((s.dot && s.epi != 1) || c11_stat_excluded(s)) return pl;
     const int MT = s.Cout_pad / 32;
     pl.MT = MT; pl.KMAX = (MT == 3 && s.Cin > 128) ? 256 : 128; pl.key = key;
     pl.tps = (int)(ft / 64);
@@ -83,7 +86,7 @@
     const int cap = pl.ny > 1 ? 256 / pl.ny + (256 % pl.ny ? 1 : 0) : 256;
     pl.gx = (int)c11_cdiv(ntiles, 8);
     if (pl.gx > cap) pl.gx = cap;
-    pl.slots = s.dot ? pl.tps : 0;
+    pl.slots = (s.dot || s.stat) ? pl.tps : 0;
     pl.family = C11_RS;
     return pl;
 }
@@ -102,9 +105,9 @@
     const int mblk = (s.Cout_pad % 128 == 0) ? 128 : ((s.Cout_pad % 64 == 0) ? 64 : ((s.Cout_pad % 96 == 0) ? 96 : 0));
     if (!mblk) return pl;
     const int tiles_t = (int)c11_cdiv(s.T, TT);
-    if (s.dot) {
+    if (s.dot || s.stat) {
         const int cpg = s.Cout / 8;
-        if (s.epi != 1 || s.x2 || gemm || (s.Cout % 8) || (cpg % 4) || (mblk % cpg) || (s.F % ROWS)) return pl;
+        if ((s.dot && (s.epi != 1 || s.x2)) || c11_stat_excluded(s) || gemm || (s.Cout % 8) || (cpg % 4) || (mblk % cpg) || (s.F % ROWS)) return pl;
         if ((int64_t)(s.F / ROWS) * tiles_t > INT32_MAX) return pl;
         pl.slots = (s.F / ROWS) * tiles_t;
     }
@@ -182,7 +185,7 @@
 static inline C11Plan c11_plan(const C11Shape& s) {
     C11Plan pl = c11_rs_plan(s);
     if (!pl.family) pl = c11_dma_plan(s);
-    if (!pl.family && (s.x2 || s.dot)) pl.ok = false;
+    if (!pl.family && (s.x2 || s.dot || s.stat)) pl.ok = false;
     else if (!pl.family) pl = c11_stream_plan(s);
     if (!pl.family && pl.ok) pl = c11_tiled_plan(s);
     return pl;
@@ -190,6 +193,6 @@
 
 template <class P> static inline C11Shape c11_shape_of(const P& p) {
     C11Shape s = {p.B, p.Cin, p.Cin1, p.Cout, p.Cout_pad, p.F, p.T, p.act, p.epi, p.in_scale != nullptr, p.res.p != nullptr, p.x2.p != nullptr, p.dot_ws != nullptr,
-                  p.ws != nullptr, p.ws_bytes};
+                  p.ws != nullptr, p.ws_bytes, p.stat_ws != nullptr};
     return s;
 }
diff --git a/audio_inpainting_diffusion_amd/csrc/aid_conv1x1_rs.hip b/audio_inpainting_diffusion_amd/csrc/aid_conv1x1_rs.hip
--- a/audio_inpainting_diffusion_amd/csrc/aid_conv1x1_rs.hip
+++ b/audio_inpainting_diffusion_amd/csrc/aid_conv1x1_rs.hip
@@ -1,6 +1,8 @@
 #include "aid_common.h"
 #include "aid_mfma_dma.h"
 #include "aid_conv1x1_plan.h"
+#include "aid_conv1x1_stat.h"
+#include "aid_fin.h"
 
 struct C11RDev {
     aid_conv2d_params p;
@@ -16,6 +18,7 @@
     constexpr int WROW = 32 * MT;
     const aid_conv2d_params& p = a.p;
     __shared__ __attribute__((aligned(16))) float wl[KMAX * WROW];
+    __shared__ double fsh[8][16];
 
     const int tid = threadIdx.x;
     const int lane = tid & 63;
@@ -98,6 +101,8 @@
         const unsigned rpos = RES ? 4u * (unsigned)(f * (int)p.res.sF + t) : 0u;
         const unsigned upos = EPI ? 4u * (unsigned)(f * (int)p.aux.sF + t) : 0u;
         float dsum[MT][4];
+        float qsum[MT][4];
+        const bool stat = !EPI && p.stat_ws != nullptr;
         int hv = half;
         asm volatile("" : "+v"(hv));
         const unsigned ys = 4u * (unsigned)p.y.sC, rs = 4u * (unsigned)p.res.sC, us = 4u * (unsigned)p.aux.sC;
@@ -109,7 +114,7 @@
         for (int i = 0; i < MT; ++i) {
             const int mbase = mb0 + 32 * i;
 #pragma unroll
-            for (int q = 0; q < 4; ++q) dsum[i][q] = 0.f;
+            for (int q = 0; q < 4; ++q) { dsum[i][q] = 0.f; qsum[i][q] = 0.f; }
             constexpr int RB = 8;
 #pragma unroll
             for (int r0 = 0; r0 < 16; r0 += RB) {
@@ -136,6 +141,7 @@
                     y0 *= p.alpha; y1 *= p.alpha;
                     *reinterpret_cast<float2*>(yb + (yo + (unsigned)(32 * i + dm) * ys)) = make_float2(y0, y1);
                     if (EPI) dsum[i][r >> 2] += y0 * uv[q].x + y1 * uv[q].y;
+                    if (stat) { dsum[i][r >> 2] += y0 + y1; qsum[i][r >> 2] += y0 * y0 + y1 * y1; }
                 }
             }
         }
@@ -157,6 +163,26 @@
                     if ((c0 + 4) / cpg == g) sacc += v1;
                 }
             if (lane < WROW / cpg && g < 8) p.dot_ws[((int64_t)be * 8 + g) * p.dot_n + tine] = (double)sacc;
+        }
+        if (stat) {
+            constexpr int CPG = 4 * MT;
+            double v1, v2;
+            const int g = c11_stat_wave<MT, CPG>(dsum, qsum, lane, v1, v2);
+            if ((lane & 7) == 0) {
+                double* o = p.stat_ws + (((int64_t)be * 8 + g) * p.stat_n + tine) * 2;
+                if (p.fin_mode) { aid_st_agent(o, v1); aid_st_agent(o + 1, v2); }
+                else { o[0] = v1; o[1] = v2; }
+            }
+            if (p.fin_mode) {
+                asm volatile("s_waitcnt vmcnt(0)" ::: "memory");
+                unsigned prev = 0;
+                if (lane == 0) prev = __hip_atomic_fetch_add(p.fin_count + be, 1u, __ATOMIC_RELAXED, __HIP_MEMORY_SCOPE_AGENT);
+                if (__builtin_amdgcn_readfirstlane(prev) == (unsigned)(a.tps - 1)) {
+                    const double n = (double)CPG * (double)p.F * (double)p.T;
+                    aid_wino_fin<true>(1, p.stat_ws, p.stat_n, be, p.Cout, n, p.fin_gamma, p.fin_mod, p.fin_mod_ld, p.fin_eps, p.fin_scale, p.fin_stats, fsh[wave], lane, 64);
+                    if (lane == 0) __hip_atomic_store(p.fin_count + be, 0u, __ATOMIC_RELAXED, __HIP_MEMORY_SCOPE_AGENT);
+                }
+            }
         }
     }
 }
@@ -199,6 +225,7 @@
     auto fits = [&](const aid_view& v, int C) { return v.sC >= 0 && v.sF >= 0 && (int64_t)4 * ((int64_t)C * v.sC + (int64_t)p->F * v.sF + p->T) < (1LL << 32); };
     if (!fits(p->x, p->Cin) || !fits(p->y, p->Cout_pad) || (p->res.p && !fits(p->res, p->Cout_pad)) || (p->aux.p && !fits(p->aux, p->Cout_pad)) || (p->x2.p && !fits(p->x2, p->Cin))) return 0;
     if (p->dot_ws && p->dot_n != pl.slots) return 0;
+    { const int rc = c11_stat_check(p, pl.slots, pl.MT); if (rc != 1) return rc; }
     int rc;
     if (pl.MT == 3) rc = pl.KMAX == 128 ? launch_c11rs<3, 128>(p, st, pl) : launch_c11rs<3, 256>(p, st, pl);
     else            rc = launch_c11rs<2, 128>(p, st, pl);
diff --git a/audio_inpainting_diffusion_amd/csrc/aid_conv1x1_stat.h b/audio_inpainting_diffusion_amd/csrc/aid_conv1x1_stat.h
--- /dev/null
+++ b/audio_inpainting_diffusion_amd/csrc/aid_conv1x1_stat.h
@@ -0,0 +1,86 @@
+#pragma once
+#include "aid_common.h"
+#include <type_traits>
+
+static constexpr bool c11_stat_geo_ok(int MT, int CPG) {
+    const int WR = 32 * MT;
+    if (CPG < 4 || (CPG % 4)) return false;
+    if (CPG > WR) return (CPG % WR) == 0;
+    const int ns = WR / CPG;
+    return (WR % CPG) == 0 && (ns == 1 || ns == 2 || ns == 4 || ns == 8);
+}
+static constexpr int c11_stat_slots(int MT, int CPG) { return CPG >= 32 * MT ? 1 : 32 * MT / CPG; }
+
+static __device__ __forceinline__ double c11_stat_pick(unsigned long long m, double a, double b) {
+    return __longlong_as_double((long long)(((unsigned long long)__double_as_longlong(a) & m) | ((unsigned long long)__double_as_longlong(b) & ~m)));
+}
+
+template <int MT, int CPG>
+static __device__ __forceinline__ int c11_stat_wave(const float (&s1)[MT][4], const float (&s2)[MT][4], int lane, double& o1, double& o2) {
+    static_assert(c11_stat_geo_ok(MT, CPG), "no (sum, sum of squares) reduction for this tile and group size");
+    constexpr int NS = c11_stat_slots(MT, CPG);
+    const bool hi = lane >= 32;
+    float g1[NS], g2[NS];
+#pragma unroll
+    for (int k = 0; k < NS; ++k) { g1[k] = 0.f; g2[k] = 0.f; }
+#pragma unroll
+    for (int i = 0; i < MT; ++i)
+#pragma unroll
+        for (int q = 0; q < 4; ++q) {
+            const int k0 = (32 * i + 8 * q) / CPG, k1 = (32 * i + 8 * q + 4) / CPG;
+            if (k0 == k1) { g1[k0] += s1[i][q]; g2[k0] += s2[i][q]; }
+            else {
+                g1[k0] += hi ? 0.f : s1[i][q]; g2[k0] += hi ? 0.f : s2[i][q];
+                g1[k1] += hi ? s1[i][q] : 0.f; g2[k1] += hi ? s2[i][q] : 0.f;
+            }
+        }
+    double d1[NS], d2[NS];
+#pragma unroll
+    for (int k = 0; k < NS; ++k) { d1[k] = (double)g1[k]; d2[k] = (double)g2[k]; }
+    int n = NS, slot = 0;
+#pragma unroll
+    for (int off = 32; off >= 1; off >>= 1) {
+        if (n > 1) {
+            n >>= 1;
+            const bool up = (lane & off) != 0;
+            const unsigned long long um = up ? ~0ull : 0ull;
+#pragma unroll
+            for (int j = 0; j < NS / 2; ++j) {
+                if (j >= n) continue;
+                const double k1 = c11_stat_pick(um, d1[j + n], d1[j]), t1 = c11_stat_pick(um, d1[j], d1[j + n]);
+                const double k2 = c11_stat_pick(um, d2[j + n], d2[j]), t2 = c11_stat_pick(um, d2[j], d2[j + n]);
+                d1[j] = k1 + __shfl_xor(t1, off, 64);
+                d2[j] = k2 + __shfl_xor(t2, off, 64);
+            }
+            slot = 2 * slot + (up ? 1 : 0);
+        } else {
+            d1[0] += __shfl_xor(d1[0], off, 64);
+            d2[0] += __shfl_xor(d2[0], off, 64);
+        }
+    }
+    o1 = d1[0]; o2 = d2[0];
+    return slot;
+}
+
+template <int MT, class F>
+static __device__ __forceinline__ void c11_stat_cpg(int cpg, F&& f) {
+#define AID_C11_STAT_CASE(v) case v: if constexpr (c11_stat_geo_ok(MT, v)) f(std::integral_constant<int, v>{}); break
+    switch (cpg) {
+        AID_C11_STAT_CASE(8); AID_C11_STAT_CASE(12); AID_C11_STAT_CASE(16); AID_C11_STAT_CASE(32); AID_C11_STAT_CASE(64); AID_C11_STAT_CASE(128);
+        default: break;
+    }
+#undef AID_C11_STAT_CASE
+}
+static inline bool c11_stat_cpg_ok(int MT, int cpg) {
+    return (cpg == 8 || cpg == 12 || cpg == 16 || cpg == 32 || cpg == 64 || cpg == 128) && c11_stat_geo_ok(MT, cpg);
+}
+
+static inline int c11_stat_check(const aid_conv2d_params* p, int slots, int MT) {
+    if (!p->stat_ws) return p->fin_mode ? 0 : 1;
+    if (slots <= 0 || p->stat_n != slots || (p->Cout % 8) || !c11_stat_cpg_ok(MT, p->Cout / 8)) return 0;
+    if (p->fin_mode && !(p->fin_mode == 1 && p->fin_count && p->fin_scale && p->fin_gamma)) {
+        aid_set_error("aid_conv2d: fin_mode on a 1x1 layer is 1 (with stat_ws) and needs fin_count, fin_scale and fin_gamma");
+        return AID_E_BADARG;
+    }
+    return 1;
+}
diff --git a/audio_inpainting_diffusion_amd/csrc/aid_fin.h b/audio_inpainting_diffusion_amd/csrc/aid_fin.h
--- a/audio_inpainting_diffusion_amd/csrc/aid_fin.h
+++ b/audio_inpainting_diffusion_amd/csrc/aid_fin.h
@@ -7,6 +7,7 @@
 static __device__ __forceinline__ void aid_st_agent(double* q, double v) {
     __hip_atomic_store(reinterpret_cast<unsigned long long*>(q), (unsigned long long)__double_as_longlong(v), __ATOMIC_RELAXED, __HIP_MEMORY_SCOPE_AGENT);
 }
+template <bool WAVE = false>
 static __device__ __attribute__((noinline)) void aid_wino_fin(int mode, const double* ws, int nk, int b, int C, double n, const float* gamma, const float* mod, int64_t mod_ld,
                                                        float eps, float* scale, float* stats, double* sh, int tid, int nthr) {
     const int lane = tid & 63, wave = tid >> 6, nw = nthr >> 6;
@@ -19,7 +20,8 @@
             for (int off = 32; off >= 1; off >>= 1) { s += __shfl_xor(s, off, 64); ss += __shfl_xor(ss, off, 64); }
             if (lane == 0) { sh[2 * g] = s; sh[2 * g + 1] = ss; }
         }
-        __syncthreads();
+        if constexpr (WAVE) __builtin_amdgcn_wave_barrier();
+        else __syncthreads();
         const int cg = C >> 3;
         for (int c = tid; c < C; c += nthr) {
             const int g = c / cg;
diff --git a/audio_inpainting_diffusion_amd/network.py b/audio_inpainting_diffusion_amd/network.py
--- a/audio_inpainting_diffusion_amd/network.py
+++ b/audio_inpainting_diffusion_amd/network.py
@@ -301,7 +301,12 @@
             self.nbytes += ws.numel() * 8
             cp.stat_ws, cp.stat_n = ws.data_ptr(), ws_n
             src[3].also_writes(ws)
-            if self.net.fuse_fin and self._fin_wanted(cp.B, src[4]) and _lib.lib().aid_conv2d_fin_supported(cp.B, cp.Cin, cp.Cout, cp.F, cp.T, cp.dilF, cp.x_wino):
+            L = _lib.lib()
+            fin_ok = (L.aid_conv2d_fin_supported_1x1(cp.B, cp.Cin, cp.Cout, cp.F, cp.T) if cp.KH == 1 else
+                      L.aid_conv2d_fin_supported(cp.B, cp.Cin, cp.Cout, cp.F, cp.T, cp.dilF, cp.x_wino))
+            if fin_ok == 2 and cp.B > 2:
+                fin_ok = 0
+            if self.net.fuse_fin and self._fin_wanted(cp.B, src[4]) and fin_ok:
                 cnt = self._fin_count(src[3].lane)
                 cp.fin_mode, cp.fin_count, cp.fin_gamma, cp.fin_eps = 1, cnt.data_ptr(), gamma.data_ptr(), 1e-7
                 cp.fin_mod, cp.fin_mod_ld = _lib.ptr(mod), (0 if mod is None else mod.stride(0))
@@ -454,8 +459,8 @@
             op = self._add("aid_conv2d", p, x, x2, y, res, wp, in_scale, out_scale, aux, aux_scale, wu, ws, dws, fin_stats, cnt, flops=2 * B * F * T * cin * cout * kh * kw,
                            nbytes=nb, writes=(y, ws, dws, cnt))
         self._wrote(y)
-        if not self._in_bwd and form and epi == 0 and dot is None and self.net.epilogue_stats:
-            n = int(_lib.lib().aid_conv2d_stat_partials(B, cin, cout, F, T, dil, fm.code))
+        if not self._in_bwd and epi == 0 and dot is None and self.net.epilogue_stats and (form or (kh == kw == 1 and x2 is None and not act)):
+            n = int(_lib.lib().aid_conv2d_stat_partials(B, cin, cout, F, T, dil, fm.code) if form else _lib.lib().aid_conv2d_stat_partials_1x1(B, cin, cout, F, T))
             if n:
                 hi = y.data_ptr() + 4 * (1 + sum((m - 1) * st for m, st in zip(y.shape, y.stride())))
                 self._stat_src[self._vkey(y)] = (p, n, hi, op, form)
diff --git a/include/aid_kernels.h b/include/aid_kernels.h
--- a/include/aid_kernels.h
+++ b/include/aid_kernels.h
@@ -64,6 +64,8 @@
 } aid_conv2d_params;
 int aid_conv2d(const aid_conv2d_params* p, void* stream);
 int aid_conv2d_dot_partials_1x1(int B, int Cin, int Cout, int F, int T);
+int aid_conv2d_stat_partials_1x1(int B, int Cin, int Cout, int F, int T);
+int aid_conv2d_fin_supported_1x1(int B, int Cin, int Cout, int F, int T);
 int aid_conv2d_x2_supported(int Cin, int Cin1, int Cout, int F, int T);
 int aid_conv2d_wino_input_supported(int Cin, int Cout, int T);
 int aid_conv2d_wino_input_ok(int B, int Cin, int Cout, int F, int T, int dilF);
```
